# openjamoses/TOSEM-2021-Replication

Hardware: AMD Instinct MI355X
Metric: train_tokens_per_s (higher is better)
Workload: dtype bf16; 1 GPU; model=mltc-base, global_batch=128, seq_len=512, parallelism=dp1

## Files before the change

### csrc/flash_attn.hip

```cpp

#include "common.h"
#include "launchers.h"

typedef __attribute__((ext_vector_type(16))) float f32x16;
typedef __attribute__((ext_vector_type(2))) unsigned uint2_t;
typedef __attribute__((ext_vector_type(4))) unsigned uint4_t;

#define FA_DH 64
#define FA_KVB 32
#define FA_QB 32
#define FA_WAVES 4
#define FA_BLOCK (FA_WAVES * WAVE)
#define FA_QWG (FA_WAVES * FA_QB)
#define FA_Q2WG (2 * FA_QWG)

#define TILE_LDS_BYTES (FA_KVB * 128)
#define FWD_LDS_BYTES (2 * TILE_LDS_BYTES + FA_WAVES * 64 * sizeof(float))
#define BWD_LDS_BYTES (2 * TILE_LDS_BYTES + 64 * sizeof(float))
#define BWD_SEG_LDS_BYTES (BWD_LDS_BYTES + 32 * sizeof(int))
#define DQ_LDS_BYTES TILE_LDS_BYTES
#define DQR_LDS_BYTES (2 * TILE_LDS_BYTES + 16)

struct FaGeom {
  long qkv_bs, qkv_hs; int qkv_rs;
  long o_bs, o_hs; int o_rs;
  static FaGeom bhld(int H, int L) {
    return {(long)H * L * FA_DH, (long)L * FA_DH, FA_DH,
            (long)H * L * FA_DH, (long)L * FA_DH, FA_DH};
  }
  static FaGeom packed(int H, int L) {
    const int D = H * FA_DH;
    return {(long)L * 3 * D, 64L, 3 * D, (long)L * D, 64L, D};
  }
};


__device__ __forceinline__ int kswz(int row, int byte_off) {
  return byte_off ^ ((row & 7) << 4);
}

__device__ __forceinline__ int c_row(int r, int half) {
  return (r & 3) + 8 * (r >> 2) + 4 * half;
}

struct FaStager {
  int row, byte;
  __device__ __forceinline__ explicit FaStager(int tid)
      : row(tid >> 3), byte((tid & 7) * 16) {}
  __device__ __forceinline__ short8_t load(const short* base, int row0,
                                           int rs) const {
    return *(const short8_t*)(base + (long)(row0 + row) * rs + (byte >> 1));
  }
  __device__ __forceinline__ void store(short* lds, short8_t v) const {
    *(short8_t*)((char*)lds + row * 128 + kswz(row, byte)) = v;
  }
};

__device__ __forceinline__ short8_t tile_row_frag(const short* lds, int col,
                                                  int half, int c) {
  return *(const short8_t*)((const char*)lds + col * 128 +
                            kswz(col, (16 * c + 8 * half) * 2));
}

__device__ __forceinline__ void cvt_pk_swap(const float (&s)[16], int r0,
                                            int r1, uint4_t& u, int i) {
  unsigned lo, hi;
  asm("v_cvt_pk_bf16_f32 %0, %1, %2\n\ts_nop 1" : "=v"(lo)
      : "v"(s[r0]), "v"(s[r0 + 1]));
  asm("v_cvt_pk_bf16_f32 %0, %1, %2\n\ts_nop 1" : "=v"(hi)
      : "v"(s[r1]), "v"(s[r1 + 1]));
  auto sw = __builtin_amdgcn_permlane32_swap(lo, hi, false, false);
  u[i] = sw[0]; u[i + 2] = sw[1];
}

__device__ __forceinline__ void c_to_afrag2(const float (&sa)[16],
                                            short8_t (&fa)[2],
                                            const float (&sb)[16],
                                            short8_t (&fb)[2]) {
#pragma unroll
  for (int c = 0; c < 2; ++c) {
    uint4_t ua, ub;
#pragma unroll
    for (int i = 0; i < 2; ++i) {
      int r0 = c * 8 + 2 * i;
      int r1 = c * 8 + 4 + 2 * i;
      cvt_pk_swap(sa, r0, r1, ua, i);
      cvt_pk_swap(sb, r0, r1, ub, i);
    }
    fa[c] = __builtin_bit_cast(short8_t, ua);
    fb[c] = __builtin_bit_cast(short8_t, ub);
  }
}

struct FaTrFrags {
  uint2_t r[8];
  __device__ __forceinline__ short8_t frag(int c, int t) const {
    uint4_t w;
    w[0] = r[c * 4 + 0 * 2 + t][0];
    w[1] = r[c * 4 + 0 * 2 + t][1];
    w[2] = r[c * 4 + 1 * 2 + t][0];
    w[3] = r[c * 4 + 1 * 2 + t][1];
    return __builtin_bit_cast(short8_t, w);
  }
};

struct FaTrOffsets { unsigned a[8]; };

__device__ __forceinline__ FaTrOffsets tr_offsets(int lane, int half) {
  const int row_mate = (lane >> 2) & 3;
  const int d_lane = 16 * ((lane >> 4) & 1) + 4 * (lane & 3);
  FaTrOffsets o;
#pragma unroll
  for (int c = 0; c < 2; ++c)
#pragma unroll
    for (int rr = 0; rr < 2; ++rr)
#pragma unroll
      for (int t = 0; t < 2; ++t) {
        int row = 16 * c + 8 * half + 4 * rr + row_mate;
        int dcol = (32 * t + d_lane) * 2;
        o.a[c * 4 + rr * 2 + t] = row * 128 + kswz(row, dcol);
      }
  return o;
}

__device__ __forceinline__ void tr_issue(const short* lds,
                                         const FaTrOffsets& o, FaTrFrags& f) {
  const unsigned base = (unsigned)(unsigned long)(char*)lds;
  unsigned a[8];
#pragma unroll
  for (int i = 0; i < 8; ++i) a[i] = base + o.a[i];
  asm volatile(
      "ds_read_b64_tr_b16 %0, %8\n\t"
      "ds_read_b64_tr_b16 %1, %9\n\t"
      "ds_read_b64_tr_b16 %2, %10\n\t"
      "ds_read_b64_tr_b16 %3, %11\n\t"
      "ds_read_b64_tr_b16 %4, %12\n\t"
      "ds_read_b64_tr_b16 %5, %13\n\t"
      "ds_read_b64_tr_b16 %6, %14\n\t"
      "ds_read_b64_tr_b16 %7, %15\n\t"
      "s_waitcnt lgkmcnt(0)"
      : "=&v"(f.r[0]), "=&v"(f.r[1]), "=&v"(f.r[2]), "=&v"(f.r[3]),
        "=&v"(f.r[4]), "=&v"(f.r[5]), "=&v"(f.r[6]), "=&v"(f.r[7])
      : "v"(a[0]), "v"(a[1]), "v"(a[2]), "v"(a[3]), "v"(a[4]), "v"(a[5]),
        "v"(a[6]), "v"(a[7])
      : "memory");
}

__device__ __forceinline__ void tr_gather(const short* lds,
                                          const FaTrOffsets& o, FaTrFrags& f) {
  tr_issue(lds, o, f);
  __builtin_amdgcn_sched_barrier(0);
}

struct FaQBlocks { int bh, qA, qB; };

__device__ __forceinline__ FaQBlocks fa_qblocks(int L, int wid) {
  const int n_qblocks = (L + FA_Q2WG - 1) / FA_Q2WG;
  const int bid = xcd_group_remap(blockIdx.x, gridDim.x, n_qblocks);
  const int qA = (bid % n_qblocks) * FA_Q2WG + wid * FA_QB;
  return {bid / n_qblocks, qA, qA + FA_QWG};
}

__device__ __forceinline__ float fa_half_merge(float s) {
  return s + __shfl_xor(s, 32, WAVE);
}

__device__ __forceinline__ void fa_colsum_merge_store(const float* cs, int tid,
                                                      float* dst0,
                                                      float* dst1) {
  if (tid < 2 * FA_DH) {
    const int slot = tid / FA_DH, c = tid % FA_DH;
    const float* p = cs + slot * FA_WAVES * FA_DH + c;
    float s = p[0];
#pragma unroll
    for (int w = 1; w < FA_WAVES; ++w) s += p[w * FA_DH];
    float* dst = slot ? dst1 : dst0;
    if (dst) dst[c] = s;
  }
}

__device__ __forceinline__ int fa_last_active_kv(const float* mrow, int L,
                                                 int tid, int* scratch) {
  if (tid == 0) *scratch = -1;
  __syncthreads();
  int loc = -1;
  for (int kv = tid; kv < L; kv += FA_BLOCK)
    if (mrow[kv] > -1.0e8f) loc = kv;
  if (loc >= 0) atomicMax(scratch, loc);
  __syncthreads();
  return *scratch;
}

#define FA_SEG_BIAS -1.0e9f

struct FaRange { int lo, hi; };

__device__ __forceinline__ FaRange fa_seg_range(const int* srow, int L,
                                                int r_lo, int r_hi, int tid,
                                                int* scratch) {
  const int s_first = srow[r_lo], s_last = srow[r_hi];
  if (tid == 0) { scratch[0] = r_lo; scratch[1] = r_hi; }
  __syncthreads();
  int lo = r_lo, hi = r_hi;
  for (int j = tid; j < L; j += FA_BLOCK) {
    const int s = srow[j];
    if (s == s_first) lo = min(lo, j);
    if (s == s_last) hi = max(hi, j);
  }
  atomicMin(&scratch[0], lo);
  atomicMax(&scratch[1], hi);
  __syncthreads();
  return {scratch[0], scratch[1]};
}

__device__ __forceinline__ bool fa_seg_tile_live(const int (&r)[16], int a,
                                                 int b) {
  bool hit = false;
#pragma unroll
  for (int i = 0; i < 16; ++i) hit |= (r[i] == a) | (r[i] == b);
  return __builtin_amdgcn_ballot_w64(hit) != 0;
}

template <bool SEG>
__global__ void __launch_bounds__(FA_BLOCK, 2)
flash_fwd_kernel(const short* __restrict__ q, const short* __restrict__ k,
                 const short* __restrict__ v, const float* __restrict__ mask,
                 const int* __restrict__ seg,
                 short* __restrict__ o, float* __restrict__ lse,
                 int B, int H, int L, float scale, FaGeom g) {
  extern __shared__ __attribute__((aligned(16))) char smem[];
  short* k_lds = (short*)smem;
  short* v_lds = (short*)(smem + TILE_LDS_BYTES);
  float* alpha_lds = (float*)(smem + 2 * TILE_LDS_BYTES);

  const int tid = threadIdx.x;
  const int lane = tid & (WAVE - 1);
  const int wid = tid / WAVE;
  const int col = lane & 31;
  const int half = lane >> 5;
  const FaTrOffsets tro = tr_offsets(lane, half);

  const FaQBlocks qb = fa_qblocks(L, wid);
  const int b = qb.bh / H;
  const int h = qb.bh % H;
  const long qkv_off = (long)b * g.qkv_bs + (long)h * g.qkv_hs;
  const long o_off = (long)b * g.o_bs + (long)h * g.o_hs;
  const int my_qA = qb.qA + col;
  const int my_qB = qb.qB + col;
  const bool validA = my_qA < L;
  const bool validB = my_qB < L;
  const float* mrow = (!SEG && mask) ? mask + (long)b * L : nullptr;
  const int* srow = SEG ? seg + (long)b * L : nullptr;
  int sqA = 0, sqB = 0;
  if constexpr (SEG) {
    sqA = srow[validA ? my_qA : L - 1];
    sqB = srow[validB ? my_qB : L - 1];
  }

  short8_t qfA[4], qfB[4];
  {
    const short* qrA = q + qkv_off + (long)(validA ? my_qA : L - 1) * g.qkv_rs;
    const short* qrB = q + qkv_off + (long)(validB ? my_qB : L - 1) * g.qkv_rs;
#pragma unroll
    for (int c = 0; c < 4; ++c) {
      qfA[c] = *(const short8_t*)(qrA + c * 16 + half * 8);
      qfB[c] = *(const short8_t*)(qrB + c * 16 + half * 8);
    }
  }

  f32x16 oA[2], oB[2];
#pragma unroll
  for (int t = 0; t < 2; ++t) { oA[t] = (f32x16)(0.f); oB[t] = (f32x16)(0.f); }
  float mA = -3.0e38f, lA = 0.f, mB = -3.0e38f, lB = 0.f;

  const int n_kv = L / FA_KVB;
  int kt_begin = 0;
  int n_kv_eff = n_kv;
  if (mrow) {
    int last = fa_last_active_kv(mrow, L, tid, (int*)alpha_lds);
    if (last >= 0) n_kv_eff = min(n_kv, last / FA_KVB + 1);
  }
  if constexpr (SEG) {
    const int q_lo = qb.qA - wid * FA_QB;
    const FaRange kr = fa_seg_range(srow, L, q_lo, min(q_lo + FA_Q2WG, L) - 1,
                                    tid, (int*)alpha_lds);
    kt_begin = kr.lo / FA_KVB;
    n_kv_eff = kr.hi / FA_KVB + 1;
  }
  const FaStager st(tid);
  short8_t kv8 = st.load(k + qkv_off, kt_begin * FA_KVB, g.qkv_rs);
  short8_t vv8 = st.load(v + qkv_off, kt_begin * FA_KVB, g.qkv_rs);
  for (int kt = kt_begin; kt < n_kv_eff; ++kt) {
    const int kv0 = kt * FA_KVB;
    __syncthreads();
    st.store(k_lds, kv8);
    st.store(v_lds, vv8);
    __syncthreads();
    if (kt + 1 < n_kv_eff) {
      kv8 = st.load(k + qkv_off, kv0 + FA_KVB, g.qkv_rs);
      vv8 = st.load(v + qkv_off, kv0 + FA_KVB, g.qkv_rs);
    }

    float mb_r[16];
    int sk_r[16];
#pragma unroll
    for (int r = 0; r < 16; ++r) {
      if constexpr (SEG) sk_r[r] = srow[kv0 + c_row(r, half)];
      else mb_r[r] = mrow ? mrow[kv0 + c_row(r, half)] : 0.f;
    }
    if constexpr (SEG) {
      if (!fa_seg_tile_live(sk_r, sqA, sqB)) continue;
    }

    f32x16 sA = (f32x16)(0.f), sB = (f32x16)(0.f);
    __builtin_amdgcn_s_setprio(1);
#pragma unroll
    for (int c = 0; c < 4; ++c) {
      short8_t kf = tile_row_frag(k_lds, col, half, c);
      sA = __builtin_amdgcn_mfma_f32_32x32x16_bf16(kf, qfA[c], sA, 0, 0, 0);
      sB = __builtin_amdgcn_mfma_f32_32x32x16_bf16(kf, qfB[c], sB, 0, 0, 0);
    }
    __builtin_amdgcn_s_setprio(0);

    float svA[16], svB[16];
    float tmaxA = -3.0e38f, tmaxB = -3.0e38f;
#pragma unroll
    for (int r = 0; r < 16; ++r) {
      float mbA, mbB;
      if constexpr (SEG) {
        mbA = sk_r[r] == sqA ? 0.f : FA_SEG_BIAS;
        mbB = sk_r[r] == sqB ? 0.f : FA_SEG_BIAS;
      } else {
        mbA = mbB = mb_r[r];
      }
      float xA = sA[r] * scale + mbA;
      float xB = sB[r] * scale + mbB;
      svA[r] = xA; svB[r] = xB;
      tmaxA = fmaxf(tmaxA, xA);
      tmaxB = fmaxf(tmaxB, xB);
    }
    tmaxA = fmaxf(tmaxA, __shfl_xor(tmaxA, 32, WAVE));
    tmaxB = fmaxf(tmaxB, __shfl_xor(tmaxB, 32, WAVE));
    float mnA = fmaxf(mA, tmaxA), mnB = fmaxf(mB, tmaxB);
    float aA = __expf(mA - mnA), aB = __expf(mB - mnB);
    float rsA = 0.f, rsB = 0.f;
#pragma unroll
    for (int r = 0; r < 16; ++r) {
      svA[r] = __expf(svA[r] - mnA);
      svB[r] = __expf(svB[r] - mnB);
      rsA += svA[r];
      rsB += svB[r];
    }
    rsA += __shfl_xor(rsA, 32, WAVE);
    rsB += __shfl_xor(rsB, 32, WAVE);
    lA = lA * aA + rsA; mA = mnA;
    lB = lB * aB + rsB; mB = mnB;

    if (__builtin_amdgcn_ballot_w64(aA != 1.f || aB != 1.f)) {
      alpha_lds[wid * 64 + col] = aA;
      alpha_lds[wid * 64 + 32 + col] = aB;
#pragma unroll
      for (int t = 0; t < 2; ++t) {
#pragma unroll
        for (int r = 0; r < 16; ++r) {
          int qrow = c_row(r, half);
          oA[t][r] *= alpha_lds[wid * 64 + qrow];
          oB[t][r] *= alpha_lds[wid * 64 + 32 + qrow];
        }
      }
    }

    short8_t pfA[2], pfB[2];
    c_to_afrag2(svA, pfA, svB, pfB);

    FaTrFrags vT;
    tr_gather(v_lds, tro, vT);
    __builtin_amdgcn_s_setprio(1);
#pragma unroll
    for (int t = 0; t < 2; ++t) {
#pragma unroll
      for (int c = 0; c < 2; ++c) {
        short8_t vf = vT.frag(c, t);
        oA[t] = __builtin_amdgcn_mfma_f32_32x32x16_bf16(pfA[c], vf, oA[t],
                                                        0, 0, 0);
        oB[t] = __builtin_amdgcn_mfma_f32_32x32x16_bf16(pfB[c], vf, oB[t],
                                                        0, 0, 0);
      }
    }
    __builtin_amdgcn_s_setprio(0);
  }

  if (lse != nullptr && half == 0) {
    if (validA) lse[(long)qb.bh * L + my_qA] = mA + __logf(lA);
    if (validB) lse[(long)qb.bh * L + my_qB] = mB + __logf(lB);
  }
  const float invA = 1.0f / lA, invB = 1.0f / lB;
#pragma unroll
  for (int r = 0; r < 16; ++r) {
    int rloc = c_row(r, half);
    float iA = __shfl(invA, rloc, WAVE);
    float iB = __shfl(invB, rloc, WAVE);
    int qA = qb.qA + rloc, qB = qb.qB + rloc;
#pragma unroll
    for (int t = 0; t < 2; ++t) {
      if (qA < L)
        o[o_off + (long)qA * g.o_rs + 32 * t + col] =
            f32_to_bf16(oA[t][r] * iA);
      if (qB < L)
        o[o_off + (long)qB * g.o_rs + 32 * t + col] =
            f32_to_bf16(oB[t][r] * iB);
    }
  }
}

static int fa_row_blocks(int B, int L, int rows_per_wg) {
  return B * ((L + rows_per_wg - 1) / rows_per_wg);
}
static dim3 fa_grid(int B, int H, int L, int rows_per_wg) {
  return dim3(H * fa_row_blocks(B, L, rows_per_wg));
}

extern "C" int flash_bias_ws_rows(int B, int L) {
  return fa_row_blocks(B, L, FA_QWG);
}

static void fa_fwd_dispatch(const short* q, const short* k, const short* v,
                            const void* mask, const void* seg, void* o,
                            void* lse, int B, int H, int L, float scale,
                            FaGeom g, hipStream_t stream) {
  const dim3 grid = fa_grid(B, H, L, FA_Q2WG);
  if (seg)
    flash_fwd_kernel<true><<<grid, FA_BLOCK, FWD_LDS_BYTES, stream>>>(
        q, k, v, nullptr, (const int*)seg, (short*)o, (float*)lse, B, H, L,
        scale, g);
  else
    flash_fwd_kernel<false><<<grid, FA_BLOCK, FWD_LDS_BYTES, stream>>>(
        q, k, v, (const float*)mask, nullptr, (short*)o, (float*)lse, B, H, L,
        scale, g);
}

extern "C" hipError_t flash_fwd_launch(const void* q, const void* k,
                                       const void* v, const void* mask,
                                       const void* seg, void* o, void* lse,
                                       int B, int H, int L, float scale,
                                       hipStream_t stream) {
  fa_fwd_dispatch((const short*)q, (const short*)k, (const short*)v, mask,
                  seg, o, lse, B, H, L, scale, FaGeom::bhld(H, L), stream);
  return hipGetLastError();
}

extern "C" hipError_t flash_fwd_packed_launch(const void* qkv,
                                              const void* mask,
                                              const void* seg, void* o,
                                              void* lse, int B, int H, int L,
                                              float scale,
                                              hipStream_t stream) {
  const int D = H * FA_DH;
  fa_fwd_dispatch((const short*)qkv, (const short*)qkv + D,
                  (const short*)qkv + 2 * D, mask, seg, o, lse, B, H, L,
                  scale, FaGeom::packed(H, L), stream);
  return hipGetLastError();
}



template <bool SEG, bool BIAS>
__global__ void __launch_bounds__(FA_BLOCK, 2)
flash_bwd_fused_kernel(const short* __restrict__ q, const short* __restrict__ k,
                       const short* __restrict__ v,
                       const short* __restrict__ dout,
                       const float* __restrict__ mask,
                       const int* __restrict__ seg,
                       const float* __restrict__ lse,
                       const float* __restrict__ ddot,
                       short* __restrict__ ds, short* __restrict__ dk,
                       short* __restrict__ dv,
                       int B, int H, int L, float scale, FaGeom g,
                       float* __restrict__ bias_ws, int bias_ld) {
  extern __shared__ __attribute__((aligned(16))) char smem[];
  short* q_lds = (short*)smem;
  short* do_lds = (short*)(smem + TILE_LDS_BYTES);
  float* lse_lds = (float*)(smem + 2 * TILE_LDS_BYTES);
  float* dd_lds = lse_lds + 32;
  int* seg_lds = (int*)(dd_lds + 32);

  const int tid = threadIdx.x;
  const int lane = tid & (WAVE - 1);
  const int wid = tid / WAVE;
  const int col = lane & 31;
  const int half = lane >> 5;
  const FaTrOffsets tro = tr_offsets(lane, half);

  const int n_kvblocks = (L + FA_QWG - 1) / FA_QWG;
  int bid = xcd_group_remap(blockIdx.x, gridDim.x, n_kvblocks);
  int bh = bid / n_kvblocks;
  int kb = bid % n_kvblocks;
  const int b = bh / H;
  const int h = bh % H;
  const long qkv_off = (long)b * g.qkv_bs + (long)h * g.qkv_hs;
  const long o_off = (long)b * g.o_bs + (long)h * g.o_hs;
  const long bh_sq = (long)bh * L * L;
  const int kv_base = kb * FA_QWG + wid * FA_KVB;
  const int my_kv = kv_base + col;
  const bool kv_valid = my_kv < L;
  const float* mrow = (!SEG && mask) ? mask + (long)b * L : nullptr;
  const float mb = mrow ? mrow[min(my_kv, L - 1)] : 0.f;
  const int* srow = SEG ? seg + (long)b * L : nullptr;
  int sk = 0;
  if constexpr (SEG) sk = srow[min(my_kv, L - 1)];

  bool skip_tile = false;
  bool wave_skip = false;
  if (mrow && ds == nullptr) {
    int* any_lds = (int*)lse_lds;
    if (tid == 0) *any_lds = 0;
    __syncthreads();
    if (kv_valid && mb > -1.0e8f) *any_lds = 1;
    __syncthreads();
    skip_tile = (*any_lds == 0) && (mrow[0] > -1.0e8f);
    __syncthreads();
    wave_skip = !skip_tile && (mrow[0] > -1.0e8f) &&
        __builtin_amdgcn_ballot_w64(kv_valid && mb > -1.0e8f) == 0;
  }

  short8_t kf[4], vf[4];
  if (!skip_tile) {
    const short* kr = k + qkv_off + (long)(kv_valid ? my_kv : L - 1) * g.qkv_rs;
    const short* vr = v + qkv_off + (long)(kv_valid ? my_kv : L - 1) * g.qkv_rs;
#pragma unroll
    for (int c = 0; c < 4; ++c) {
      kf[c] = *(const short8_t*)(kr + c * 16 + half * 8);
      vf[c] = *(const short8_t*)(vr + c * 16 + half * 8);
    }
  }
  f32x16 dv_acc[2], dk_acc[2];
#pragma unroll
  for (int t = 0; t < 2; ++t) {
    dv_acc[t] = (f32x16)(0.f);
    dk_acc[t] = (f32x16)(0.f);
  }
  if (!skip_tile) {
  int qt_begin = 0;
  int n_q = L / 32;
  if constexpr (SEG) {
    const int kv_lo = kb * FA_QWG;
    const FaRange qr = fa_seg_range(srow, L, kv_lo, min(kv_lo + FA_QWG, L) - 1,
                                    tid, (int*)lse_lds);
    qt_begin = qr.lo / 32;
    n_q = qr.hi / 32 + 1;
  }
  const FaStager st(tid);
  short8_t qv8 = st.load(q + qkv_off, qt_begin * 32, g.qkv_rs);
  short8_t dv8 = st.load(dout + o_off, qt_begin * 32, g.o_rs);
  for (int qt = qt_begin; qt < n_q; ++qt) {
    const int q0 = qt * 32;
    __syncthreads();
    st.store(q_lds, qv8);
    st.store(do_lds, dv8);
    if (tid < 32) {
      lse_lds[tid] = lse[(long)bh * L + q0 + tid];
      dd_lds[tid] = ddot[(long)bh * L + q0 + tid];
      if constexpr (SEG) seg_lds[tid] = srow[q0 + tid];
    }
    __syncthreads();
    if (qt + 1 < n_q) {
      qv8 = st.load(q + qkv_off, q0 + 32, g.qkv_rs);
      dv8 = st.load(dout + o_off, q0 + 32, g.o_rs);
    }

    if (wave_skip) continue;
    int sq_r[16];
    if constexpr (SEG) {
#pragma unroll
      for (int r = 0; r < 16; ++r) sq_r[r] = seg_lds[c_row(r, half)];
      if (!fa_seg_tile_live(sq_r, sk, sk)) continue;
    }
    f32x16 s_acc = (f32x16)(0.f);
    f32x16 dp_acc = (f32x16)(0.f);
    __builtin_amdgcn_s_setprio(1);
#pragma unroll
    for (int c = 0; c < 4; ++c) {
      short8_t qfrag = tile_row_frag(q_lds, col, half, c);
      short8_t dofrag = tile_row_frag(do_lds, col, half, c);
      s_acc = __builtin_amdgcn_mfma_f32_32x32x16_bf16(qfrag, kf[c], s_acc,
                                                      0, 0, 0);
      dp_acc = __builtin_amdgcn_mfma_f32_32x32x16_bf16(dofrag, vf[c], dp_acc,
                                                       0, 0, 0);
    }
    __builtin_amdgcn_s_setprio(0);

    float pv[16], gv[16];
#pragma unroll
    for (int r = 0; r < 16; ++r) {
      int ql = c_row(r, half);
      float bias = mb;
      if constexpr (SEG) bias = sq_r[r] == sk ? 0.f : FA_SEG_BIAS;
      pv[r] = __expf(s_acc[r] * scale + bias - lse_lds[ql]);
      gv[r] = scale * pv[r] * (dp_acc[r] - dd_lds[ql]);
    }
    if (!SEG && ds != nullptr && kv_valid) {
#pragma unroll
      for (int r = 0; r < 16; ++r)
        ds[bh_sq + (long)(q0 + c_row(r, half)) * L + my_kv] =
            f32_to_bf16(gv[r]);
    }

    short8_t pf[2], gf[2];
    c_to_afrag2(pv, pf, gv, gf);

    FaTrFrags doT, qT;
    tr_issue(do_lds, tro, doT);
    tr_gather(q_lds, tro, qT);
    __builtin_amdgcn_s_setprio(1);
#pragma unroll
    for (int t = 0; t < 2; ++t) {
#pragma unroll
      for (int c = 0; c < 2; ++c) {
        dv_acc[t] = __builtin_amdgcn_mfma_f32_32x32x16_bf16(
            pf[c], doT.frag(c, t), dv_acc[t], 0, 0, 0);
        dk_acc[t] = __builtin_amdgcn_mfma_f32_32x32x16_bf16(
            gf[c], qT.frag(c, t), dk_acc[t], 0, 0, 0);
      }
    }
    __builtin_amdgcn_s_setprio(0);
  }
  }

  float csk[2] = {0.f, 0.f}, csv[2] = {0.f, 0.f};
#pragma unroll
  for (int t = 0; t < 2; ++t) {
#pragma unroll
    for (int r = 0; r < 16; ++r) {
      int kvl = c_row(r, half);
      if (kv_base + kvl >= L) continue;
      long off = qkv_off + (long)(kv_base + kvl) * g.qkv_rs + 32 * t + col;
      const short vb = f32_to_bf16(dv_acc[t][r]);
      const short kb16 = f32_to_bf16(dk_acc[t][r]);
      dv[off] = vb;
      dk[off] = kb16;
      if constexpr (BIAS) {
        csv[t] += bf16_to_f32(vb);
        csk[t] += bf16_to_f32(kb16);
      }
    }
  }
  if constexpr (BIAS) {
    float* cs = (float*)smem;
    __syncthreads();
#pragma unroll
    for (int t = 0; t < 2; ++t) {
      float sk_ = fa_half_merge(csk[t]);
      float sv_ = fa_half_merge(csv[t]);
      if (half == 0) {
        cs[(0 * FA_WAVES + wid) * FA_DH + 32 * t + col] = sk_;
        cs[(1 * FA_WAVES + wid) * FA_DH + 32 * t + col] = sv_;
      }
    }
    __syncthreads();
    const int third = bias_ld / 3;
    float* row = bias_ws + ((long)b * n_kvblocks + kb) * bias_ld + h * FA_DH;
    fa_colsum_merge_store(cs, tid, row + third, row + 2 * third);
  }
}

static void fa_bwd_fused_dispatch(const short* q, const short* k,
                                  const short* v, const void* dout,
                                  const void* mask, const void* seg,
                                  const void* lse, const void* ddot, void* ds,
                                  short* dk, short* dv, int B, int H, int L,
                                  float scale, FaGeom g, float* bias_ws,
                                  hipStream_t stream) {
  const dim3 grid = fa_grid(B, H, L, FA_QWG);
  const int bias_ld = 3 * H * FA_DH;
#define FA_BWD_SEG_ARGS                                                       \
  q, k, v, (const short*)dout, nullptr, (const int*)seg, (const float*)lse,   \
      (const float*)ddot, nullptr, dk, dv, B, H, L, scale, g, bias_ws, bias_ld
#define FA_BWD_ARGS                                                           \
  q, k, v, (const short*)dout, (const float*)mask, nullptr,                   \
      (const float*)lse, (const float*)ddot, (short*)ds, dk, dv, B, H, L,     \
      scale, g, bias_ws, bias_ld
  if (seg && bias_ws) {
    flash_bwd_fused_kernel<true, true><<<grid, FA_BLOCK, BWD_SEG_LDS_BYTES,
                                         stream>>>(FA_BWD_SEG_ARGS);
  } else if (seg) {
    flash_bwd_fused_kernel<true, false><<<grid, FA_BLOCK, BWD_SEG_LDS_BYTES,
                                          stream>>>(FA_BWD_SEG_ARGS);
  } else if (bias_ws) {
    flash_bwd_fused_kernel<false, true><<<grid, FA_BLOCK, BWD_LDS_BYTES,
                                          stream>>>(FA_BWD_ARGS);
  } else {
    flash_bwd_fused_kernel<false, false><<<grid, FA_BLOCK, BWD_LDS_BYTES,
                                           stream>>>(FA_BWD_ARGS);
  }
#undef FA_BWD_ARGS
#undef FA_BWD_SEG_ARGS
}

extern "C" hipError_t flash_bwd_fused_launch(
    const void* q, const void* k, const void* v, const void* dout,
    const void* mask, const void* seg, const void* lse, const void* ddot,
    void* ds, void* dk, void* dv, int B, int H, int L, float scale,
    hipStream_t stream) {
  if (seg && ds) return hipErrorInvalidValue;
  fa_bwd_fused_dispatch((const short*)q, (const short*)k, (const short*)v,
                        dout, mask, seg, lse, ddot, ds, (short*)dk,
                        (short*)dv, B, H, L, scale, FaGeom::bhld(H, L),
                        nullptr, stream);
  return hipGetLastError();
}

extern "C" hipError_t flash_bwd_fused_packed_launch(
    const void* qkv, const void* dout, const void* mask, const void* seg,
    const void* lse, const void* ddot, void* dqkv, void* bias_ws, int B,
    int H, int L, float scale, hipStream_t stream) {
  const int D = H * FA_DH;
  fa_bwd_fused_dispatch((const short*)qkv, (const short*)qkv + D,
                        (const short*)qkv + 2 * D, dout, mask, seg, lse, ddot,
                        nullptr, (short*)dqkv + D, (short*)dqkv + 2 * D, B, H,
                        L, scale, FaGeom::packed(H, L), (float*)bias_ws,
                        stream);
  return hipGetLastError();
}

extern "C" __global__ void __launch_bounds__(FA_BLOCK, 2)
flash_dq_kernel(const short* __restrict__ ds, const short* __restrict__ k,
                short* __restrict__ dq, int B, int H, int L) {
  extern __shared__ __attribute__((aligned(16))) char smem[];
  short* k_lds = (short*)smem;

  const int tid = threadIdx.x;
  const int lane = tid & (WAVE - 1);
  const int wid = tid / WAVE;
  const int col = lane & 31;
  const int half = lane >> 5;
  const FaTrOffsets tro = tr_offsets(lane, half);

  const FaQBlocks qb = fa_qblocks(L, wid);
  const long bh_off = (long)qb.bh * L * FA_DH;
  const long bh_sq = (long)qb.bh * L * L;
  const int my_qA = min(qb.qA + col, L - 1);
  const int my_qB = min(qb.qB + col, L - 1);
  const short* dsA_row = ds + bh_sq + (long)my_qA * L;
  const short* dsB_row = ds + bh_sq + (long)my_qB * L;

  f32x16 oA[2], oB[2];
#pragma unroll
  for (int t = 0; t < 2; ++t) { oA[t] = (f32x16)(0.f); oB[t] = (f32x16)(0.f); }

  const int n_kv = L / FA_KVB;
  const FaStager st(tid);
  short8_t kv8 = st.load(k + bh_off, 0, FA_DH);
  for (int kt = 0; kt < n_kv; ++kt) {
    const int kv0 = kt * FA_KVB;
    __syncthreads();
    st.store(k_lds, kv8);
    __syncthreads();
    if (kt + 1 < n_kv) kv8 = st.load(k + bh_off, kv0 + FA_KVB, FA_DH);
    short8_t aA[2], aB[2];
#pragma unroll
    for (int c = 0; c < 2; ++c) {
      aA[c] = *(const short8_t*)(dsA_row + kv0 + 16 * c + 8 * half);
      aB[c] = *(const short8_t*)(dsB_row + kv0 + 16 * c + 8 * half);
    }
    FaTrFrags kT;
    tr_gather(k_lds, tro, kT);
    __builtin_amdgcn_s_setprio(1);
#pragma unroll
    for (int t = 0; t < 2; ++t) {
#pragma unroll
      for (int c = 0; c < 2; ++c) {
        short8_t kf = kT.frag(c, t);
        oA[t] = __builtin_amdgcn_mfma_f32_32x32x16_bf16(aA[c], kf, oA[t],
                                                        0, 0, 0);
        oB[t] = __builtin_amdgcn_mfma_f32_32x32x16_bf16(aB[c], kf, oB[t],
                                                        0, 0, 0);
      }
    }
    __builtin_amdgcn_s_setprio(0);
  }

#pragma unroll
  for (int t = 0; t < 2; ++t) {
#pragma unroll
    for (int r = 0; r < 16; ++r) {
      int rloc = c_row(r, half);
      int qA = qb.qA + rloc, qB = qb.qB + rloc;
      if (qA < L)
        dq[bh_off + (long)qA * FA_DH + 32 * t + col] = f32_to_bf16(oA[t][r]);
      if (qB < L)
        dq[bh_off + (long)qB * FA_DH + 32 * t + col] = f32_to_bf16(oB[t][r]);
    }
  }
}

extern "C" hipError_t flash_dq_launch(const void* ds, const void* k, void* dq,
                                      int B, int H, int L,
                                      hipStream_t stream) {
  flash_dq_kernel<<<fa_grid(B, H, L, FA_Q2WG), FA_BLOCK, DQ_LDS_BYTES,
                    stream>>>(
      (const short*)ds, (const short*)k, (short*)dq, B, H, L);
  return hipGetLastError();
}

template <bool SEG, bool BIAS>
__global__ void __launch_bounds__(FA_BLOCK, 2)
flash_dq_recompute_kernel(const short* __restrict__ q,
                          const short* __restrict__ k,
                          const short* __restrict__ v,
                          const short* __restrict__ dout,
                          const float* __restrict__ mask,
                          const int* __restrict__ seg,
                          const float* __restrict__ lse,
                          const float* __restrict__ ddot,
                          short* __restrict__ dq,
                          int B, int H, int L, float scale, FaGeom g,
                          float* __restrict__ bias_ws, int bias_ld) {
  extern __shared__ __attribute__((aligned(16))) char smem[];
  short* k_lds = (short*)smem;
  short* v_lds = (short*)(smem + TILE_LDS_BYTES);
  int* skip_scratch = (int*)(smem + 2 * TILE_LDS_BYTES);

  const int tid = threadIdx.x;
  const int lane = tid & (WAVE - 1);
  const int wid = tid / WAVE;
  const int col = lane & 31;
  const int half = lane >> 5;
  const FaTrOffsets tro = tr_offsets(lane, half);

  const FaQBlocks qb = fa_qblocks(L, wid);
  const int b = qb.bh / H;
  const int h = qb.bh % H;
  const long qkv_off = (long)b * g.qkv_bs + (long)h * g.qkv_hs;
  const long o_off = (long)b * g.o_bs + (long)h * g.o_hs;
  const int my_qA = qb.qA + col;
  const int my_qB = qb.qB + col;
  const bool validA = my_qA < L;
  const bool validB = my_qB < L;
  const float* mrow = (!SEG && mask) ? mask + (long)b * L : nullptr;
  const int* srow = SEG ? seg + (long)b * L : nullptr;
  int sqA = 0, sqB = 0;
  if constexpr (SEG) {
    sqA = srow[validA ? my_qA : L - 1];
    sqB = srow[validB ? my_qB : L - 1];
  }

  short8_t qfA[4], qfB[4], dofA[4], dofB[4];
  {
    const short* qrA = q + qkv_off + (long)(validA ? my_qA : L - 1) * g.qkv_rs;
    const short* qrB = q + qkv_off + (long)(validB ? my_qB : L - 1) * g.qkv_rs;
    const short* drA = dout + o_off + (long)(validA ? my_qA : L - 1) * g.o_rs;
    const short* drB = dout + o_off + (long)(validB ? my_qB : L - 1) * g.o_rs;
#pragma unroll
    for (int c = 0; c < 4; ++c) {
      qfA[c] = *(const short8_t*)(qrA + c * 16 + half * 8);
      qfB[c] = *(const short8_t*)(qrB + c * 16 + half * 8);
      dofA[c] = *(const short8_t*)(drA + c * 16 + half * 8);
      dofB[c] = *(const short8_t*)(drB + c * 16 + half * 8);
    }
  }
  const float lseA = lse[(long)qb.bh * L + (validA ? my_qA : L - 1)];
  const float lseB = lse[(long)qb.bh * L + (validB ? my_qB : L - 1)];
  const float ddA = ddot[(long)qb.bh * L + (validA ? my_qA : L - 1)];
  const float ddB = ddot[(long)qb.bh * L + (validB ? my_qB : L - 1)];

  f32x16 dqA[2], dqB[2];
#pragma unroll
  for (int t = 0; t < 2; ++t) { dqA[t] = (f32x16)(0.f); dqB[t] = (f32x16)(0.f); }

  const int n_kv = L / FA_KVB;
  int kt_begin = 0;
  int n_kv_eff = n_kv;
  if (mrow) {
    int last = fa_last_active_kv(mrow, L, tid, skip_scratch);
    if (last >= 0) n_kv_eff = min(n_kv, last / FA_KVB + 1);
  }
  if constexpr (SEG) {
    const int q_lo = qb.qA - wid * FA_QB;
    const FaRange kr = fa_seg_range(srow, L, q_lo, min(q_lo + FA_Q2WG, L) - 1,
                                    tid, skip_scratch);
    kt_begin = kr.lo / FA_KVB;
    n_kv_eff = kr.hi / FA_KVB + 1;
  }
  const FaStager st(tid);
  short8_t kv8 = st.load(k + qkv_off, kt_begin * FA_KVB, g.qkv_rs);
  short8_t vv8 = st.load(v + qkv_off, kt_begin * FA_KVB, g.qkv_rs);
  for (int kt = kt_begin; kt < n_kv_eff; ++kt) {
    const int kv0 = kt * FA_KVB;
    __syncthreads();
    st.store(k_lds, kv8);
    st.store(v_lds, vv8);
    __syncthreads();
    if (kt + 1 < n_kv_eff) {
      kv8 = st.load(k + qkv_off, kv0 + FA_KVB, g.qkv_rs);
      vv8 = st.load(v + qkv_off, kv0 + FA_KVB, g.qkv_rs);
    }

    float mb_r[16];
    int sk_r[16];
#pragma unroll
    for (int r = 0; r < 16; ++r) {
      if constexpr (SEG) sk_r[r] = srow[kv0 + c_row(r, half)];
      else mb_r[r] = mrow ? mrow[kv0 + c_row(r, half)] : 0.f;
    }
    if constexpr (SEG) {
      if (!fa_seg_tile_live(sk_r, sqA, sqB)) continue;
    }

    f32x16 sA = (f32x16)(0.f), sB = (f32x16)(0.f);
    f32x16 pA = (f32x16)(0.f), pB = (f32x16)(0.f);
    __builtin_amdgcn_s_setprio(1);
#pragma unroll
    for (int c = 0; c < 4; ++c) {
      short8_t kf = tile_row_frag(k_lds, col, half, c);
      short8_t vf = tile_row_frag(v_lds, col, half, c);
      sA = __builtin_amdgcn_mfma_f32_32x32x16_bf16(kf, qfA[c], sA, 0, 0, 0);
      sB = __builtin_amdgcn_mfma_f32_32x32x16_bf16(kf, qfB[c], sB, 0, 0, 0);
      pA = __builtin_amdgcn_mfma_f32_32x32x16_bf16(vf, dofA[c], pA, 0, 0, 0);
      pB = __builtin_amdgcn_mfma_f32_32x32x16_bf16(vf, dofB[c], pB, 0, 0, 0);
    }
    __builtin_amdgcn_s_setprio(0);

    float gA[16], gB[16];
#pragma unroll
    for (int r = 0; r < 16; ++r) {
      float mbA, mbB;
      if constexpr (SEG) {
        mbA = sk_r[r] == sqA ? 0.f : FA_SEG_BIAS;
        mbB = sk_r[r] == sqB ? 0.f : FA_SEG_BIAS;
      } else {
        mbA = mbB = mb_r[r];
      }
      float expA = __expf(sA[r] * scale + mbA - lseA);
      float expB = __expf(sB[r] * scale + mbB - lseB);
      gA[r] = scale * expA * (pA[r] - ddA);
      gB[r] = scale * expB * (pB[r] - ddB);
    }

    short8_t gfA[2], gfB[2];
    c_to_afrag2(gA, gfA, gB, gfB);

    FaTrFrags kT;
    tr_gather(k_lds, tro, kT);
    __builtin_amdgcn_s_setprio(1);
#pragma unroll
    for (int t = 0; t < 2; ++t) {
#pragma unroll
      for (int c = 0; c < 2; ++c) {
        short8_t kf = kT.frag(c, t);
        dqA[t] = __builtin_amdgcn_mfma_f32_32x32x16_bf16(gfA[c], kf, dqA[t],
                                                         0, 0, 0);
        dqB[t] = __builtin_amdgcn_mfma_f32_32x32x16_bf16(gfB[c], kf, dqB[t],
                                                         0, 0, 0);
      }
    }
    __builtin_amdgcn_s_setprio(0);
  }

  float csA[2] = {0.f, 0.f}, csB[2] = {0.f, 0.f};
#pragma unroll
  for (int t = 0; t < 2; ++t) {
#pragma unroll
    for (int r = 0; r < 16; ++r) {
      int rloc = c_row(r, half);
      int qA = qb.qA + rloc, qB = qb.qB + rloc;
      if (qA < L) {
        const short a16 = f32_to_bf16(dqA[t][r]);
        dq[qkv_off + (long)qA * g.qkv_rs + 32 * t + col] = a16;
        if constexpr (BIAS) csA[t] += bf16_to_f32(a16);
      }
      if (qB < L) {
        const short b16 = f32_to_bf16(dqB[t][r]);
        dq[qkv_off + (long)qB * g.qkv_rs + 32 * t + col] = b16;
        if constexpr (BIAS) csB[t] += bf16_to_f32(b16);
      }
    }
  }
  if constexpr (BIAS) {
    float* cs = (float*)smem;
    __syncthreads();
#pragma unroll
    for (int t = 0; t < 2; ++t) {
      float sA_ = fa_half_merge(csA[t]);
      float sB_ = fa_half_merge(csB[t]);
      if (half == 0) {
        cs[(0 * FA_WAVES + wid) * FA_DH + 32 * t + col] = sA_;
        cs[(1 * FA_WAVES + wid) * FA_DH + 32 * t + col] = sB_;
      }
    }
    __syncthreads();
    const int n128 = (L + FA_QWG - 1) / FA_QWG;
    const int blkA = (qb.qA - wid * FA_QB) / FA_QWG;
    float* row = bias_ws + ((long)b * n128 + blkA) * bias_ld + h * FA_DH;
    fa_colsum_merge_store(cs, tid, row,
                          blkA + 1 < n128 ? row + bias_ld : nullptr);
  }
}

static void fa_dq_recompute_dispatch(const short* q, const short* k,
                                     const short* v, const void* dout,
                                     const void* mask, const void* seg,
                                     const void* lse, const void* ddot,
                                     void* dq, int B, int H, int L,
                                     float scale, FaGeom g, float* bias_ws,
                                     hipStream_t stream) {
  const dim3 grid = fa_grid(B, H, L, FA_Q2WG);
  const int bias_ld = 3 * H * FA_DH;
#define FA_DQR_SEG_ARGS                                                       \
  q, k, v, (const short*)dout, nullptr, (const int*)seg, (const float*)lse,   \
      (const float*)ddot, (short*)dq, B, H, L, scale, g, bias_ws, bias_ld
#define FA_DQR_ARGS                                                           \
  q, k, v, (const short*)dout, (const float*)mask, nullptr,                   \
      (const float*)lse, (const float*)ddot, (short*)dq, B, H, L, scale, g,   \
      bias_ws, bias_ld
  if (seg && bias_ws) {
    flash_dq_recompute_kernel<true, true><<<grid, FA_BLOCK, DQR_LDS_BYTES,
                                            stream>>>(FA_DQR_SEG_ARGS);
  } else if (seg) {
    flash_dq_recompute_kernel<true, false><<<grid, FA_BLOCK, DQR_LDS_BYTES,
                                             stream>>>(FA_DQR_SEG_ARGS);
  } else if (bias_ws) {
    flash_dq_recompute_kernel<false, true><<<grid, FA_BLOCK, DQR_LDS_BYTES,
                                             stream>>>(FA_DQR_ARGS);
  } else {
    flash_dq_recompute_kernel<false, false><<<grid, FA_BLOCK, DQR_LDS_BYTES,
                                              stream>>>(FA_DQR_ARGS);
  }
#undef FA_DQR_ARGS
#undef FA_DQR_SEG_ARGS
}

extern "C" hipError_t flash_dq_recompute_launch(
    const void* q, const void* k, const void* v, const void* dout,
    const void* mask, const void* seg, const void* lse, const void* ddot,
    void* dq, int B, int H, int L, float scale, hipStream_t stream) {
  fa_dq_recompute_dispatch((const short*)q, (const short*)k, (const short*)v,
                           dout, mask, seg, lse, ddot, dq, B, H, L, scale,
                           FaGeom::bhld(H, L), nullptr, stream);
  return hipGetLastError();
}

extern "C" hipError_t flash_dq_recompute_packed_launch(
    const void* qkv, const void* dout, const void* mask, const void* seg,
    const void* lse, const void* ddot, void* dqkv, void* bias_ws, int B,
    int H, int L, float scale, hipStream_t stream) {
  const int D = H * FA_DH;
  fa_dq_recompute_dispatch((const short*)qkv, (const short*)qkv + D,
                           (const short*)qkv + 2 * D, dout, mask, seg, lse,
                           ddot, dqkv, B, H, L, scale, FaGeom::packed(H, L),
                           (float*)bias_ws, stream);
  return hipGetLastError();
}

__device__ __forceinline__ float fa_row_dot(const short* dr, const short* orow,
                                            int sub) {
  short4_t a = *(const short4_t*)(dr + sub * 4);
  short4_t c = *(const short4_t*)(orow + sub * 4);
  float s = 0.f;
#pragma unroll
  for (int j = 0; j < 4; ++j) s += bf16_to_f32(a[j]) * bf16_to_f32(c[j]);
#pragma unroll
  for (int off = 8; off > 0; off >>= 1) s += __shfl_xor(s, off, 16);
  return s;
}

extern "C" __global__ void __launch_bounds__(256)
fa_dot_kernel(const short* __restrict__ dout, const short* __restrict__ o,
              float* __restrict__ ddot, long n_rows) {
  long row = ((long)blockIdx.x * 256 + threadIdx.x) >> 4;
  if (row >= n_rows) return;
  int sub = threadIdx.x & 15;
  float s = fa_row_dot(dout + row * FA_DH, o + row * FA_DH, sub);
  if (sub == 0) ddot[row] = s;
}

extern "C" __global__ void __launch_bounds__(256)
fa_dot_packed_kernel(const short* __restrict__ dout,
                     const short* __restrict__ o, float* __restrict__ ddot,
                     int B, int H, int L) {
  const int D = H * FA_DH;
  long n_rows = (long)B * L * H;
  long chunk = ((long)blockIdx.x * 256 + threadIdx.x) >> 4;
  if (chunk >= n_rows) return;
  int sub = threadIdx.x & 15;
  int h = (int)(chunk % H);
  long bl = chunk / H;
  int l = (int)(bl % L);
  int b = (int)(bl / L);
  float s = fa_row_dot(dout + bl * D + h * FA_DH, o + bl * D + h * FA_DH, sub);
  if (sub == 0) ddot[((long)b * H + h) * L + l] = s;
}

extern "C" hipError_t fa_dot_packed_launch(const void* dout, const void* o,
                                           void* ddot, int B, int H, int L,
                                           hipStream_t stream) {
  long total_threads = (long)B * H * L * 16;
  int grid = (int)((total_threads + 255) / 256);
  fa_dot_packed_kernel<<<grid, 256, 0, stream>>>(
      (const short*)dout, (const short*)o, (float*)ddot, B, H, L);
  return hipGetLastError();
}

extern "C" hipError_t fa_dot_launch(const void* dout, const void* o,
                                    void* ddot, long n_rows,
                                    hipStream_t stream) {
  long total_threads = n_rows * 16;
  int grid = (int)((total_threads + 255) / 256);
  fa_dot_kernel<<<grid, 256, 0, stream>>>((const short*)dout, (const short*)o,
                                          (float*)ddot, n_rows);
  return hipGetLastError();
}

extern "C" __global__ void __launch_bounds__(64)
tr_probe_kernel(const short* __restrict__ src, short* __restrict__ out,
                int scheme) {
  __shared__ __attribute__((aligned(16))) short lds[256];
  int lane = threadIdx.x;
  for (int i = lane; i < 256; i += 64) lds[i] = src[i];
  __syncthreads();
  int addr;
  switch (scheme) {
    case 0: addr = 0; break;
    case 1: addr = (lane & 15) * 2; break;
    case 2: addr = ((lane & 15) + (lane >> 4) * 64) * 2; break;
    case 3: addr = (lane >> 4) * 128; break;
    case 4: addr = (lane & 3) * 16; break;
    case 5: addr = ((lane & 3) * 32 + 4 * ((lane >> 2) & 7)) * 2; break;
    case 6: addr = ((lane & 3) * 8 + 4) * 2; break;
    case 7: addr = ((lane & 3) == 0) ? 16 : 0; break;
    case 8: addr = ((lane & 3) == 1) ? 16 : 0; break;
    case 9: addr = ((lane & 3) == 2) ? 16 : 0; break;
    case 10: addr = ((lane & 3) == 3) ? 16 : 0; break;
    case 11: addr = ((lane & 3) * 64 + 4 * ((lane >> 2) & 7)) * 2; break;
    default: addr = ((lane & 3) * 8 + ((lane >> 2) & 7) * 32) * 2; break;
  }
  typedef __attribute__((ext_vector_type(2))) unsigned uint2_t;
  uint2_t r;
  unsigned base = (unsigned)(unsigned long)((char*)lds + addr);
  asm volatile("ds_read_b64_tr_b16 %0, %1\n\ts_waitcnt lgkmcnt(0)"
               : "=v"(r) : "v"(base) : "memory");
  __builtin_amdgcn_sched_barrier(0);
  out[lane * 4 + 0] = (short)(r[0] & 0xffff);
  out[lane * 4 + 1] = (short)(r[0] >> 16);
  out[lane * 4 + 2] = (short)(r[1] & 0xffff);
  out[lane * 4 + 3] = (short)(r[1] >> 16);
}

extern "C" hipError_t tr_probe_launch(const void* src, void* out, int scheme,
                                      hipStream_t stream) {
  tr_probe_kernel<<<1, 64, 0, stream>>>((const short*)src, (short*)out,
                                        scheme);
  return hipGetLastError();
}
```

### csrc/launchers.h

```cpp
#pragma once

#include <hip/hip_runtime.h>

extern "C" {

hipError_t ln_fwd_launch(const void* x, const void* res, const void* gamma,
                         const void* beta, void* y, void* s_out, void* mean,
                         void* rstd, int N, int D, float eps,
                         hipStream_t stream);
hipError_t ln_bwd_launch(const void* dy, const void* x, const void* gamma,
                         const void* mean, const void* rstd,
                         const void* ds_extra, void* dx, void* ws, int n_out,
                         int N, int D, hipStream_t stream);
int ln_bwd_ws_rows(int N, int D);
hipError_t ln_drop_fwd_launch(const void* x, const void* res,
                              const void* gamma, const void* beta, void* y,
                              void* s_out, void* mean, void* rstd, int N,
                              int D, float eps, unsigned long long seed,
                              unsigned call, unsigned site, unsigned thr,
                              hipStream_t stream);
hipError_t ln_drop_bwd_launch(const void* dy, const void* x,
                              const void* gamma, const void* mean,
                              const void* rstd, const void* ds_extra, void* dx,
                              void* dres, void* ws, int N, int D,
                              unsigned long long seed, unsigned call,
                              unsigned site, unsigned thr,
                              hipStream_t stream);
int ln_drop_bwd_max_d(void);

hipError_t colsum_launch(const void* ws, void* scratch, void* out, int R,
                         int D, int split_w, int out_bf16,
                         hipStream_t stream);
int colsum_scratch_rows(void);
hipError_t colsum_bf16_launch(const void* x, void* scratch, void* out, long N,
                              int D, hipStream_t stream);
int colsum_bf16_scratch_rows(void);

hipError_t bias_gelu_fwd_launch(const void* x, const void* b, void* y,
                                long n_elem, int D, hipStream_t stream);
hipError_t bias_gelu_bwd_launch(const void* dy, const void* x, const void* b,
                                void* dx, void* ws_dbias, long n_elem, int D,
                                hipStream_t stream);
int bias_gelu_bwd_ws_rows(long n_elem, int D);

hipError_t softmax_fwd_launch(const void* s, const void* mask, void* p,
                              long n_rows, int Lk, int H_Lq, float scale,
                              hipStream_t stream);
hipError_t softmax_bwd_launch(const void* dp, const void* p, void* ds,
                              long n_rows, int Lk, float scale,
                              hipStream_t stream);
hipError_t p_from_lse_launch(const void* s, const void* mask, const void* lse,
                             void* p, long n_rows, int Lk, int H_Lq,
                             float scale, hipStream_t stream);

hipError_t adamw_launch(void* p_bf16, const void* grad, int grad_is_f32,
                        void* m, void* v, void* master, long n, float lr,
                        float beta1, float beta2, float eps, float wd,
                        int step, float grad_scale, hipStream_t stream);
hipError_t adamw_clipped_launch(void* p_bf16, const void* grad,
                                int grad_is_f32, void* m, void* v,
                                void* master, long n, float lr, float beta1,
                                float beta2, float eps, float wd, int step,
                                const void* clip_state, hipStream_t stream);
hipError_t grad_clip_state_launch(const void* grad, int grad_is_f32, long n,
                                  float grad_scale, float max_norm,
                                  void* partials, void* clip_state,
                                  hipStream_t stream);
int grad_norm_grid(long n);

hipError_t qkv_repack_launch(const void* src, void* dst, int B, int L, int H,
                             int dh, int backward, hipStream_t stream);
hipError_t qkv_repack_bwd3_launch(const void* dq, const void* dk,
                                  const void* dv, void* dsrc, int B, int L,
                                  int H, int dh, hipStream_t stream);
hipError_t out_repack_launch(const void* src, void* dst, int B, int L, int H,
                             int dh, int backward, hipStream_t stream);

hipError_t flash_fwd_launch(const void* q, const void* k, const void* v,
                            const void* mask, const void* seg, void* o,
                            void* lse, int B, int H, int L, float scale,
                            hipStream_t stream);
hipError_t flash_fwd_packed_launch(const void* qkv, const void* mask,
                                   const void* seg, void* o, void* lse, int B,
                                   int H, int L, float scale,
                                   hipStream_t stream);
hipError_t flash_bwd_fused_launch(const void* q, const void* k, const void* v,
                                  const void* dout, const void* mask,
                                  const void* seg, const void* lse,
                                  const void* ddot, void* ds, void* dk,
                                  void* dv, int B, int H, int L, float scale,
                                  hipStream_t stream);
hipError_t flash_bwd_fused_packed_launch(const void* qkv, const void* dout,
                                         const void* mask, const void* seg,
                                         const void* lse, const void* ddot,
                                         void* dqkv, void* bias_ws, int B,
                                         int H, int L, float scale,
                                         hipStream_t stream);
hipError_t flash_dq_recompute_packed_launch(const void* qkv, const void* dout,
                                            const void* mask, const void* seg,
                                            const void* lse, const void* ddot,
                                            void* dqkv, void* bias_ws, int B,
                                            int H, int L, float scale,
                                            hipStream_t stream);
int flash_bias_ws_rows(int B, int L);
hipError_t flash_dq_recompute_launch(const void* q, const void* k,
                                     const void* v, const void* dout,
                                     const void* mask, const void* seg,
                                     const void* lse, const void* ddot,
                                     void* dq, int B, int H, int L,
                                     float scale, hipStream_t stream);
hipError_t flash_dq_launch(const void* ds, const void* k, void* dq, int B,
                           int H, int L, hipStream_t stream);
hipError_t fa_dot_launch(const void* dout, const void* o, void* ddot,
                         long n_rows, hipStream_t stream);
hipError_t fa_dot_packed_launch(const void* dout, const void* o, void* ddot,
                                int B, int H, int L, hipStream_t stream);
hipError_t tr_probe_launch(const void* src, void* out, int scheme,
                           hipStream_t stream);

hipError_t masked_pool_fwd_launch(const void* x, const void* mask,
                                  void* pooled, void* counts, void* ws, int B,
                                  int L, int D, hipStream_t stream);
int masked_pool_ws_splits(void);
hipError_t masked_pool_bwd_launch(const void* dpooled, const void* mask,
                                  const void* counts, void* dx, int B, int L,
                                  int D, hipStream_t stream);
hipError_t segment_pool_fwd_launch(const void* x, const void* seg_start,
                                   const void* seg_len, void* pooled, int N,
                                   long T, int D, hipStream_t stream);
hipError_t segment_pool_bwd_launch(const void* dpooled, const void* pos2seg,
                                   const void* seg_len, void* dx, int N,
                                   long T, int D, hipStream_t stream);

hipError_t wgrad_gemm_launch(const void* a, const void* b, void* ws, void* out,
                             int M, int N, long K, int S, hipStream_t stream);

}
```

### csrc/ops.cpp

```cpp

#include <torch/extension.h>
#include <c10/hip/HIPStream.h>
#include <hip/hip_runtime.h>

#include "launchers.h"
#include "lt_gemm.h"

namespace {

#define CHECK_HIP(call)                                                   \
  do {                                                                    \
    hipError_t e_ = (call);                                               \
    TORCH_CHECK(e_ == hipSuccess, "HIP error: ", hipGetErrorString(e_));  \
  } while (0)

hipStream_t cur_stream() {
  return c10::hip::getCurrentHIPStream().stream();
}

void check_bf16(const torch::Tensor& t, const char* name) {
  TORCH_CHECK(t.is_contiguous(), name, " must be contiguous");
  TORCH_CHECK(t.scalar_type() == torch::kBFloat16, name, " must be bf16");
  TORCH_CHECK(t.device().is_cuda(), name, " must be on GPU");
}

void check_f32(const torch::Tensor& t, const char* name) {
  TORCH_CHECK(t.is_contiguous(), name, " must be contiguous");
  TORCH_CHECK(t.scalar_type() == torch::kFloat32, name, " must be f32");
  TORCH_CHECK(t.device().is_cuda(), name, " must be on GPU");
}

void check_shape(const torch::Tensor& t, const char* name,
                 at::IntArrayRef want, const char* shape) {
  TORCH_CHECK(t.sizes() == want, name, " must be ", shape);
}

void check_numel(const torch::Tensor& t, const char* name, long n,
                 const char* shape) {
  TORCH_CHECK(t.numel() == n, name, " must be ", shape);
}

void check_mult8(long v, const char* name) {
  TORCH_CHECK(v % 8 == 0, name, " must be a multiple of 8, got ", v);
}

const void* softmax_mask_ptr(const c10::optional<torch::Tensor>& mask,
                             const torch::Tensor& scores, int* H_Lq) {
  *H_Lq = 1;
  if (!mask.has_value()) return nullptr;
  check_f32(*mask, "mask");
  TORCH_CHECK(scores.dim() == 4, "masked scores must be [B, H, Lq, Lk]");
  check_shape(*mask, "mask", {scores.size(0), scores.size(3)}, "[B, Lk]");
  *H_Lq = (int)(scores.size(1) * scores.size(2));
  return mask->data_ptr();
}

const void* pool_mask_ptr(const c10::optional<torch::Tensor>& mask,
                          const torch::Tensor& x, long B, long L) {
  if (!mask.has_value()) return nullptr;
  TORCH_CHECK(mask->scalar_type() == torch::kBool && mask->is_contiguous(),
              "mask must be contiguous bool");
  TORCH_CHECK(mask->device() == x.device(), "mask must be on the same device "
              "as the data");
  check_shape(*mask, "mask", {B, L}, "[B, L]");
  return mask->data_ptr();
}

torch::Tensor colsum(const torch::Tensor& ws, long split_w, bool out_bf16) {
  const long R = ws.size(0), W = ws.size(1);
  auto out = torch::empty(
      {W}, out_bf16 ? ws.options().dtype(torch::kBFloat16) : ws.options());
  auto scratch = torch::empty({colsum_scratch_rows(), W}, ws.options());
  CHECK_HIP(colsum_launch(ws.data_ptr(), scratch.data_ptr(), out.data_ptr(),
                          (int)R, (int)W, (int)split_w, out_bf16 ? 1 : 0,
                          cur_stream()));
  return out;
}


struct FlashDims { long B, H, L; };
using NamedTensor = std::pair<const char*, torch::Tensor>;

const void* flash_mask_ptr(const c10::optional<torch::Tensor>& mask,
                           const FlashDims& d) {
  if (!mask.has_value()) return nullptr;
  check_f32(*mask, "mask");
  TORCH_CHECK(mask->dim() == 2 && mask->size(0) == d.B &&
              mask->size(1) == d.L, "mask must be [B, L]");
  return mask->data_ptr();
}

const void* flash_seg_ptr(const c10::optional<torch::Tensor>& seg,
                          const c10::optional<torch::Tensor>& mask,
                          const torch::Tensor& x, const FlashDims& d) {
  if (!seg.has_value()) return nullptr;
  TORCH_CHECK(!mask.has_value(), "mask and seg are mutually exclusive");
  TORCH_CHECK(seg->scalar_type() == torch::kInt32, "seg must be int32");
  TORCH_CHECK(seg->device() == x.device(), "seg must be on the same device "
              "as the attention inputs");
  TORCH_CHECK(seg->is_contiguous(), "seg must be contiguous");
  TORCH_CHECK(seg->dim() == 2 && seg->size(0) == d.B && seg->size(1) == d.L,
              "seg must be [B, L]");
  return seg->data_ptr();
}

void check_i32(const torch::Tensor& t, const torch::Tensor& like,
               const char* name) {
  TORCH_CHECK(t.is_contiguous(), name, " must be contiguous");
  TORCH_CHECK(t.scalar_type() == torch::kInt32, name, " must be int32");
  TORCH_CHECK(t.device() == like.device(), name, " must be on the same "
              "device as the data");
}

void check_flash_rows(std::initializer_list<NamedTensor> rows,
                      const FlashDims& d) {
  for (const auto& [name, t] : rows) {
    check_f32(t, name);
    TORCH_CHECK(t.dim() == 3 && t.size(0) == d.B && t.size(1) == d.H &&
                t.size(2) == d.L, name, " must be [B, H, L]");
  }
}

FlashDims check_flash_bhld(const char* xname, const torch::Tensor& x,
                           std::initializer_list<NamedTensor> same,
                           std::initializer_list<NamedTensor> rows) {
  check_bf16(x, xname);
  TORCH_CHECK(x.dim() == 4, xname, " must be [B, H, L, 64]");
  const FlashDims d{x.size(0), x.size(1), x.size(2)};
  TORCH_CHECK(x.size(3) == 64, "flash kernels are specialized for head_dim 64");
  TORCH_CHECK(d.L % 32 == 0, "flash kernels need L % 32 == 0");
  for (const auto& [name, t] : same) {
    check_bf16(t, name);
    TORCH_CHECK(t.sizes() == x.sizes(), name, " must match ", xname,
                "'s shape");
  }
  check_flash_rows(rows, d);
  return d;
}

FlashDims check_flash_packed(const torch::Tensor& qkv, long H,
                             std::initializer_list<NamedTensor> outs,
                             std::initializer_list<NamedTensor> rows) {
  check_bf16(qkv, "qkv");
  TORCH_CHECK(qkv.dim() == 3, "qkv must be [B, L, 3D]");
  const FlashDims d{qkv.size(0), H, qkv.size(1)};
  TORCH_CHECK(qkv.size(2) == 3 * H * 64, "qkv last dim must be 3*H*64");
  TORCH_CHECK(d.L % 32 == 0, "flash kernels need L % 32 == 0");
  for (const auto& [name, t] : outs) {
    check_bf16(t, name);
    TORCH_CHECK(t.dim() == 3 && t.size(0) == d.B && t.size(1) == d.L &&
                t.size(2) == H * 64, name, " must be [B, L, H*64]");
  }
  check_flash_rows(rows, d);
  return d;
}

}

std::vector<torch::Tensor> layernorm_fwd(torch::Tensor x,
                                         c10::optional<torch::Tensor> residual,
                                         torch::Tensor gamma,
                                         torch::Tensor beta, double eps) {
  check_bf16(x, "x"); check_bf16(gamma, "gamma"); check_bf16(beta, "beta");
  const int D = (int)x.size(-1);
  const long N = x.numel() / D;
  TORCH_CHECK(D % 8 == 0, "D must be a multiple of 8, got ", D);
  check_numel(gamma, "gamma", D, "[D]");
  check_numel(beta, "beta", D, "[D]");
  if (residual.has_value()) {
    check_bf16(*residual, "residual");
    TORCH_CHECK(residual->sizes() == x.sizes(), "residual shape mismatch");
  }
  auto y = torch::empty_like(x);
  auto opts = x.options().dtype(torch::kFloat32);
  auto mean = torch::empty({N}, opts);
  auto rstd = torch::empty({N}, opts);
  const void* res_ptr = nullptr;
  torch::Tensor s_out;
  void* s_ptr = nullptr;
  if (residual.has_value()) {
    res_ptr = residual->data_ptr();
    s_out = torch::empty_like(x);
    s_ptr = s_out.data_ptr();
  } else {
    s_out = x;
  }
  CHECK_HIP(ln_fwd_launch(x.data_ptr(), res_ptr, gamma.data_ptr(),
                          beta.data_ptr(), y.data_ptr(), s_ptr,
                          mean.data_ptr(), rstd.data_ptr(), (int)N, D,
                          (float)eps, cur_stream()));
  return {y, s_out, mean, rstd};
}

std::vector<torch::Tensor> layernorm_bwd(torch::Tensor dy, torch::Tensor x,
                                         torch::Tensor gamma, torch::Tensor mean,
                                         torch::Tensor rstd,
                                         c10::optional<torch::Tensor> ds_extra,
                                         bool want_dres, bool out_bf16) {
  check_bf16(dy, "dy"); check_bf16(x, "x"); check_bf16(gamma, "gamma");
  const int D = (int)x.size(-1);
  const long N = x.numel() / D;
  TORCH_CHECK(D % 8 == 0, "D must be a multiple of 8, got ", D);
  TORCH_CHECK(dy.numel() == x.numel(), "dy shape mismatch");
  check_numel(gamma, "gamma", D, "[D]");
  check_f32(mean, "mean"); check_f32(rstd, "rstd");
  TORCH_CHECK(mean.numel() == N && rstd.numel() == N,
              "mean and rstd must be [N]");
  const void* de = nullptr;
  if (ds_extra.has_value()) {
    check_bf16(*ds_extra, "ds_extra");
    TORCH_CHECK(ds_extra->numel() == x.numel(), "ds_extra shape mismatch");
    de = ds_extra->data_ptr();
  }
  auto dx = torch::empty_like(x);
  const int n_out = want_dres ? 3 : 2;
  auto ws = torch::empty({ln_bwd_ws_rows((int)N, D), n_out * D},
                         x.options().dtype(torch::kFloat32));
  CHECK_HIP(ln_bwd_launch(dy.data_ptr(), x.data_ptr(), gamma.data_ptr(),
                          mean.data_ptr(), rstd.data_ptr(), de, dx.data_ptr(),
                          ws.data_ptr(), n_out, (int)N, D, cur_stream()));
  auto cols = colsum(ws, 2 * D, out_bf16);
  std::vector<torch::Tensor> out = {dx, cols.narrow(0, 0, D),
                                    cols.narrow(0, D, D)};
  if (want_dres) out.push_back(cols.narrow(0, 2 * D, D));
  return out;
}

void check_drop_args(int64_t call, int64_t site, int64_t thr) {
  TORCH_CHECK(call >= 0 && call <= 0xffffffffLL, "call must fit 32 bits");
  TORCH_CHECK(site >= 0 && site <= 0xffffffffLL, "site must fit 32 bits");
  TORCH_CHECK(thr >= 1 && thr <= 65535,
              "dropout threshold must be in [1, 65535], got ", thr);
}

std::vector<torch::Tensor> layernorm_drop_fwd(torch::Tensor x,
                                              torch::Tensor residual,
                                              torch::Tensor gamma,
                                              torch::Tensor beta, double eps,
                                              uint64_t seed, int64_t call,
                                              int64_t site, int64_t thr) {
  check_bf16(x, "x"); check_bf16(gamma, "gamma"); check_bf16(beta, "beta");
  check_bf16(residual, "residual");
  const int D = (int)x.size(-1);
  const long N = x.numel() / D;
  TORCH_CHECK(D % 8 == 0, "D must be a multiple of 8, got ", D);
  check_numel(gamma, "gamma", D, "[D]");
  check_numel(beta, "beta", D, "[D]");
  TORCH_CHECK(residual.sizes() == x.sizes(), "residual shape mismatch");
  TORCH_CHECK(D <= ln_drop_bwd_max_d(), "fused dropout LayerNorm supports "
              "D <= ", ln_drop_bwd_max_d(), ", got ", D);
  check_drop_args(call, site, thr);
  auto y = torch::empty_like(x);
  auto s_out = torch::empty_like(x);
  auto opts = x.options().dtype(torch::kFloat32);
  auto mean = torch::empty({N}, opts);
  auto rstd = torch::empty({N}, opts);
  CHECK_HIP(ln_drop_fwd_launch(x.data_ptr(), residual.data_ptr(),
                               gamma.data_ptr(), beta.data_ptr(), y.data_ptr(),
                               s_out.data_ptr(), mean.data_ptr(),
                               rstd.data_ptr(), (int)N, D, (float)eps, seed,
                               (unsigned)call, (unsigned)site, (unsigned)thr,
                               cur_stream()));
  return {y, s_out, mean, rstd};
}

std::vector<torch::Tensor> layernorm_drop_bwd(
    torch::Tensor dy, torch::Tensor x, torch::Tensor gamma, torch::Tensor mean,
    torch::Tensor rstd, c10::optional<torch::Tensor> ds_extra, bool out_bf16,
    uint64_t seed, int64_t call, int64_t site, int64_t thr) {
  check_bf16(dy, "dy"); check_bf16(x, "x"); check_bf16(gamma, "gamma");
  const int D = (int)x.size(-1);
  const long N = x.numel() / D;
  TORCH_CHECK(D % 8 == 0, "D must be a multiple of 8, got ", D);
  TORCH_CHECK(D <= ln_drop_bwd_max_d(), "fused dropout LayerNorm backward "
              "supports D <= ", ln_drop_bwd_max_d(), ", got ", D);
  TORCH_CHECK(dy.numel() == x.numel(), "dy shape mismatch");
  check_numel(gamma, "gamma", D, "[D]");
  check_f32(mean, "mean"); check_f32(rstd, "rstd");
  TORCH_CHECK(mean.numel() == N && rstd.numel() == N,
              "mean and rstd must be [N]");
  check_drop_args(call, site, thr);
  const void* de = nullptr;
  if (ds_extra.has_value()) {
    check_bf16(*ds_extra, "ds_extra");
    TORCH_CHECK(ds_extra->numel() == x.numel(), "ds_extra shape mismatch");
    de = ds_extra->data_ptr();
  }
  auto dx = torch::empty_like(x);
  auto dres = torch::empty_like(x);
  auto ws = torch::empty({ln_bwd_ws_rows((int)N, D), 2 * D},
                         x.options().dtype(torch::kFloat32));
  CHECK_HIP(ln_drop_bwd_launch(dy.data_ptr(), x.data_ptr(), gamma.data_ptr(),
                               mean.data_ptr(), rstd.data_ptr(), de,
                               dx.data_ptr(), dres.data_ptr(), ws.data_ptr(),
                               (int)N, D, seed, (unsigned)call, (unsigned)site,
                               (unsigned)thr, cur_stream()));
  auto cols = colsum(ws, 2 * D, out_bf16);
  return {dx, dres, cols.narrow(0, 0, D), cols.narrow(0, D, D)};
}

torch::Tensor bias_gelu_fwd(torch::Tensor x, torch::Tensor b) {
  check_bf16(x, "x"); check_bf16(b, "b");
  const int D = (int)x.size(-1);
  const long n = x.numel();
  TORCH_CHECK(D % 8 == 0, "D must be a multiple of 8");
  check_numel(b, "b", D, "[D]");
  auto y = torch::empty_like(x);
  CHECK_HIP(bias_gelu_fwd_launch(x.data_ptr(), b.data_ptr(), y.data_ptr(), n,
                                 D, cur_stream()));
  return y;
}

std::vector<torch::Tensor> bias_gelu_bwd(torch::Tensor dy, torch::Tensor x,
                                         torch::Tensor b, bool out_bf16) {
  check_bf16(dy, "dy"); check_bf16(x, "x"); check_bf16(b, "b");
  const int D = (int)x.size(-1);
  const long n = x.numel();
  TORCH_CHECK(D % 8 == 0, "D must be a multiple of 8");
  check_numel(b, "b", D, "[D]");
  TORCH_CHECK(dy.numel() == x.numel(), "dy shape mismatch");
  auto dx = torch::empty_like(x);
  auto ws = torch::empty({bias_gelu_bwd_ws_rows(n, D), D},
                         x.options().dtype(torch::kFloat32));
  CHECK_HIP(bias_gelu_bwd_launch(dy.data_ptr(), x.data_ptr(), b.data_ptr(),
                                 dx.data_ptr(), ws.data_ptr(), n, D,
                                 cur_stream()));
  return {dx, colsum(ws, D, out_bf16)};
}

torch::Tensor softmax_fwd(torch::Tensor scores, c10::optional<torch::Tensor> mask,
                          double scale) {
  check_bf16(scores, "scores");
  const int Lk = (int)scores.size(-1);
  const long n_rows = scores.numel() / Lk;
  check_mult8(Lk, "Lk");
  int H_Lq;
  const void* mptr = softmax_mask_ptr(mask, scores, &H_Lq);
  auto p = torch::empty_like(scores);
  CHECK_HIP(softmax_fwd_launch(scores.data_ptr(), mptr, p.data_ptr(), n_rows,
                               Lk, H_Lq, (float)scale, cur_stream()));
  return p;
}

torch::Tensor softmax_bwd(torch::Tensor dp, torch::Tensor p, double scale) {
  check_bf16(dp, "dp"); check_bf16(p, "p");
  const int Lk = (int)p.size(-1);
  const long n_rows = p.numel() / Lk;
  check_mult8(Lk, "Lk");
  TORCH_CHECK(dp.sizes() == p.sizes(), "dp must match p's shape");
  auto ds = torch::empty_like(p);
  CHECK_HIP(softmax_bwd_launch(dp.data_ptr(), p.data_ptr(), ds.data_ptr(),
                               n_rows, Lk, (float)scale, cur_stream()));
  return ds;
}

void adamw_step(torch::Tensor p, torch::Tensor grad, torch::Tensor m,
                torch::Tensor v, torch::Tensor master, double lr, double beta1,
                double beta2, double eps, double wd, long step,
                double grad_scale) {
  check_bf16(p, "p"); check_f32(m, "m"); check_f32(v, "v");
  check_f32(master, "master");
  TORCH_CHECK(grad.is_contiguous() && grad.device().is_cuda(), "bad grad");
  int gf32 = grad.scalar_type() == torch::kFloat32;
  TORCH_CHECK(gf32 || grad.scalar_type() == torch::kBFloat16,
              "grad must be f32 or bf16");
  const long n = p.numel();
  TORCH_CHECK(n % 4 == 0, "flat parameter buffer must be padded to 4 elems");
  TORCH_CHECK(grad.numel() == n && m.numel() == n && v.numel() == n &&
              master.numel() == n, "size mismatch");
  CHECK_HIP(adamw_launch(p.data_ptr(), grad.data_ptr(), gf32, m.data_ptr(),
                         v.data_ptr(), master.data_ptr(), n, (float)lr,
                         (float)beta1, (float)beta2, (float)eps, (float)wd,
                         (int)step, (float)grad_scale, cur_stream()));
}

int check_flat_grad(const torch::Tensor& grad) {
  TORCH_CHECK(grad.is_contiguous() && grad.device().is_cuda(), "bad grad");
  int gf32 = grad.scalar_type() == torch::kFloat32;
  TORCH_CHECK(gf32 || grad.scalar_type() == torch::kBFloat16,
              "grad must be f32 or bf16");
  TORCH_CHECK(grad.numel() > 0 && grad.numel() % 8 == 0,
              "flat gradient buffer must be padded to 8 elems");
  TORCH_CHECK(reinterpret_cast<uintptr_t>(grad.data_ptr()) % 16 == 0,
              "flat gradient buffer must be 16-byte aligned");
  return gf32;
}

torch::Tensor grad_clip_state(torch::Tensor grad, double grad_scale,
                              double max_norm) {
  int gf32 = check_flat_grad(grad);
  TORCH_CHECK(max_norm > 0, "max_norm must be greater than 0");
  const long n = grad.numel();
  auto opts = torch::TensorOptions().dtype(torch::kFloat32)
                  .device(grad.device());
  auto partials = torch::empty({grad_norm_grid(n)}, opts);
  auto state = torch::empty({4}, opts);
  CHECK_HIP(grad_clip_state_launch(grad.data_ptr(), gf32, n,
                                   (float)grad_scale, (float)max_norm,
                                   partials.data_ptr(), state.data_ptr(),
                                   cur_stream()));
  return state;
}

void adamw_step_clipped(torch::Tensor p, torch::Tensor grad, torch::Tensor m,
                        torch::Tensor v, torch::Tensor master, double lr,
                        double beta1, double beta2, double eps, double wd,
                        long step, torch::Tensor clip_state) {
  check_bf16(p, "p"); check_f32(m, "m"); check_f32(v, "v");
  check_f32(master, "master"); check_f32(clip_state, "clip_state");
  int gf32 = check_flat_grad(grad);
  TORCH_CHECK(clip_state.numel() == 4, "clip_state must hold 4 floats");
  const long n = p.numel();
  TORCH_CHECK(grad.numel() == n && m.numel() == n && v.numel() == n &&
              master.numel() == n, "size mismatch");
  CHECK_HIP(adamw_clipped_launch(p.data_ptr(), grad.data_ptr(), gf32,
                                 m.data_ptr(), v.data_ptr(),
                                 master.data_ptr(), n, (float)lr,
                                 (float)beta1, (float)beta2, (float)eps,
                                 (float)wd, (int)step, clip_state.data_ptr(),
                                 cur_stream()));
}

torch::Tensor qkv_repack(torch::Tensor qkv, long H, bool backward) {
  check_bf16(qkv, "qkv");
  TORCH_CHECK(H > 0, "H must be positive");
  long B, L, dh;
  if (!backward) {
    TORCH_CHECK(qkv.dim() == 3 || qkv.dim() == 5,
                "qkv must be [B, L, 3*H*dh] or [B, L, 3, H, dh]");
    B = qkv.size(0); L = qkv.size(1);
    if (qkv.dim() == 3) {
      TORCH_CHECK(qkv.size(2) % (3 * H) == 0,
                  "qkv last dim must divide evenly by 3*H");
      dh = qkv.size(2) / (3 * H);
    } else {
      check_shape(qkv, "qkv", {B, L, 3, H, qkv.size(4)}, "[B, L, 3, H, dh]");
      dh = qkv.size(4);
    }
  } else {
    TORCH_CHECK(qkv.dim() == 5, "qkv grad must be [3, B, H, L, dh]");
    B = qkv.size(1); L = qkv.size(3);
    dh = qkv.size(4);
    check_shape(qkv, "qkv grad", {3, B, H, L, dh}, "[3, B, H, L, dh]");
  }
  check_mult8(dh, "head_dim");
  auto out = backward ? torch::empty({B, L, 3 * H * dh}, qkv.options())
                      : torch::empty({3, B, H, L, dh}, qkv.options());
  CHECK_HIP(qkv_repack_launch(qkv.data_ptr(), out.data_ptr(), (int)B, (int)L,
                              (int)H, (int)dh, backward ? 1 : 0,
                              cur_stream()));
  return out;
}

torch::Tensor qkv_repack_bwd3(torch::Tensor dq, torch::Tensor dk,
                              torch::Tensor dv) {
  check_bf16(dq, "dq"); check_bf16(dk, "dk"); check_bf16(dv, "dv");
  TORCH_CHECK(dq.dim() == 4, "dq must be [B, H, L, dh]");
  TORCH_CHECK(dk.sizes() == dq.sizes(), "dk must match dq's shape");
  TORCH_CHECK(dv.sizes() == dq.sizes(), "dv must match dq's shape");
  long B = dq.size(0), H = dq.size(1), L = dq.size(2), dh = dq.size(3);
  check_mult8(dh, "head_dim");
  auto out = torch::empty({B, L, 3 * H * dh}, dq.options());
  CHECK_HIP(qkv_repack_bwd3_launch(dq.data_ptr(), dk.data_ptr(), dv.data_ptr(),
                                   out.data_ptr(), (int)B, (int)L, (int)H,
                                   (int)dh, cur_stream()));
  return out;
}

torch::Tensor out_repack(torch::Tensor x, bool backward) {
  check_bf16(x, "x");
  TORCH_CHECK(!backward,
              "pass the 4-D grad with explicit dims via out_repack_bwd");
  TORCH_CHECK(x.dim() == 4, "x must be [B, H, L, dh]");
  long B = x.size(0), H = x.size(1), L = x.size(2), dh = x.size(3);
  check_mult8(dh, "head_dim");
  auto out = torch::empty({B, L, H * dh}, x.options());
  CHECK_HIP(out_repack_launch(x.data_ptr(), out.data_ptr(), (int)B, (int)L,
                              (int)H, (int)dh, 0, cur_stream()));
  return out;
}

torch::Tensor out_repack_bwd(torch::Tensor dgrad, long H) {
  check_bf16(dgrad, "dgrad");
  TORCH_CHECK(dgrad.dim() == 3, "dgrad must be [B, L, H*dh]");
  TORCH_CHECK(H > 0 && dgrad.size(2) % H == 0,
              "dgrad last dim must divide evenly by H");
  long B = dgrad.size(0), L = dgrad.size(1), dh = dgrad.size(2) / H;
  check_mult8(dh, "head_dim");
  auto out = torch::empty({B, H, L, dh}, dgrad.options());
  CHECK_HIP(out_repack_launch(dgrad.data_ptr(), out.data_ptr(), (int)B,
                              (int)L, (int)H, (int)dh, 1, cur_stream()));
  return out;
}

std::vector<torch::Tensor> flash_fwd(torch::Tensor q, torch::Tensor k,
                                     torch::Tensor v,
                                     c10::optional<torch::Tensor> mask,
                                     double scale,
                                     c10::optional<torch::Tensor> seg) {
  const auto [B, H, L] = check_flash_bhld("q", q, {{"k", k}, {"v", v}}, {});
  const void* mptr = flash_mask_ptr(mask, {B, H, L});
  const void* sptr = flash_seg_ptr(seg, mask, q, {B, H, L});
  auto o = torch::empty_like(q);
  auto lse = torch::empty({B, H, L}, q.options().dtype(torch::kFloat32));
  CHECK_HIP(flash_fwd_launch(q.data_ptr(), k.data_ptr(), v.data_ptr(), mptr,
                             sptr, o.data_ptr(), lse.data_ptr(), (int)B,
                             (int)H, (int)L, (float)scale, cur_stream()));
  return {o, lse};
}

torch::Tensor p_from_lse(torch::Tensor scores, c10::optional<torch::Tensor> mask,
                         torch::Tensor lse, double scale) {
  check_bf16(scores, "scores"); check_f32(lse, "lse");
  const int Lk = (int)scores.size(-1);
  const long n_rows = scores.numel() / Lk;
  TORCH_CHECK(lse.numel() == n_rows, "lse size mismatch");
  check_mult8(Lk, "Lk");
  int H_Lq;
  const void* mptr = softmax_mask_ptr(mask, scores, &H_Lq);
  auto p = torch::empty_like(scores);
  CHECK_HIP(p_from_lse_launch(scores.data_ptr(), mptr, lse.data_ptr(),
                              p.data_ptr(), n_rows, Lk, H_Lq, (float)scale,
                              cur_stream()));
  return p;
}

torch::Tensor fa_dot(torch::Tensor dout, torch::Tensor o) {
  check_bf16(dout, "dout"); check_bf16(o, "o");
  TORCH_CHECK(dout.dim() == 4 && o.sizes() == dout.sizes(),
              "dout and o must both be [B, H, L, 64]");
  const long n_rows = dout.numel() / dout.size(-1);
  TORCH_CHECK(dout.size(-1) == 64, "fa_dot expects head_dim 64");
  auto d = torch::empty({n_rows}, dout.options().dtype(torch::kFloat32));
  CHECK_HIP(fa_dot_launch(dout.data_ptr(), o.data_ptr(), d.data_ptr(), n_rows,
                          cur_stream()));
  return d.view({dout.size(0), dout.size(1), dout.size(2)});
}

std::vector<torch::Tensor> flash_bwd_fused(torch::Tensor q, torch::Tensor k,
                                           torch::Tensor v, torch::Tensor dout,
                                           c10::optional<torch::Tensor> mask,
                                           torch::Tensor lse,
                                           torch::Tensor ddot, double scale,
                                           bool emit_ds,
                                           c10::optional<torch::Tensor> seg) {
  const auto [B, H, L] = check_flash_bhld(
      "q", q, {{"k", k}, {"v", v}, {"dout", dout}},
      {{"lse", lse}, {"ddot", ddot}});
  const void* mptr = flash_mask_ptr(mask, {B, H, L});
  const void* sptr = flash_seg_ptr(seg, mask, q, {B, H, L});
  TORCH_CHECK(!(sptr && emit_ds), "seg with emit_ds=True is not supported: "
              "the flash_dq A/B path is unsegmented");
  auto dk = torch::empty_like(k);
  auto dv = torch::empty_like(v);
  torch::Tensor ds;
  void* ds_ptr = nullptr;
  if (emit_ds) {
    ds = torch::empty({B, H, L, L}, q.options());
    ds_ptr = ds.data_ptr();
  }
  CHECK_HIP(flash_bwd_fused_launch(q.data_ptr(), k.data_ptr(), v.data_ptr(),
                                   dout.data_ptr(), mptr, sptr,
                                   lse.data_ptr(), ddot.data_ptr(), ds_ptr,
                                   dk.data_ptr(), dv.data_ptr(), (int)B,
                                   (int)H, (int)L, (float)scale,
                                   cur_stream()));
  if (emit_ds) return {ds, dk, dv};
  return {dk, dv};
}

torch::Tensor wgrad_gemm(torch::Tensor dy, torch::Tensor x,
                         long splits) {
  check_bf16(dy, "dy"); check_bf16(x, "x");
  TORCH_CHECK(dy.dim() == 2 && x.dim() == 2, "2-D operands required");
  const long K = dy.size(0), M = dy.size(1), N = x.size(1);
  TORCH_CHECK(x.size(0) == K, "K mismatch");
  TORCH_CHECK(M % 256 == 0 && N % 256 == 0, "M, N must be 256-multiples");
  TORCH_CHECK(K % 32 == 0, "K must be a 32-multiple");
  int S = (int)splits;
  if (S <= 0) {
    long tiles = (M / 256) * (N / 256);
    S = 1;
    while (S < 32 && tiles * S < 512 && (K / (2L * S)) % 32 == 0) S *= 2;
  }
  TORCH_CHECK((K / S) % 32 == 0, "K/S must be a 32-multiple");
  auto ws = torch::empty({S, M, N}, dy.options().dtype(torch::kFloat32));
  auto out = torch::empty({M, N}, dy.options());
  CHECK_HIP(wgrad_gemm_launch(dy.data_ptr(), x.data_ptr(), ws.data_ptr(),
                              out.data_ptr(), (int)M, (int)N, K, S,
                              cur_stream()));
  return out;
}

torch::Tensor bias_grad(torch::Tensor dy) {
  check_bf16(dy, "dy");
  const int D = (int)dy.size(-1);
  const long N = dy.numel() / D;
  TORCH_CHECK(dy.dim() == 2, "dy must be [N, D]");
  TORCH_CHECK(D % 8 == 0, "D % 8 == 0 required");
  auto scratch = torch::empty({colsum_bf16_scratch_rows(), D},
                              dy.options().dtype(torch::kFloat32));
  auto out = torch::empty({D}, dy.options());
  CHECK_HIP(colsum_bf16_launch(dy.data_ptr(), scratch.data_ptr(),
                               out.data_ptr(), N, D, cur_stream()));
  return out;
}

std::vector<torch::Tensor> flash_fwd_packed(torch::Tensor qkv, long H,
                                            c10::optional<torch::Tensor> mask,
                                            double scale,
                                            c10::optional<torch::Tensor> seg) {
  const auto dims = check_flash_packed(qkv, H, {}, {});
  const long B = dims.B, L = dims.L;
  const void* mptr = flash_mask_ptr(mask, dims);
  const void* sptr = flash_seg_ptr(seg, mask, qkv, dims);
  auto o = torch::empty({B, L, H * 64}, qkv.options());
  auto lse = torch::empty({B, H, L}, qkv.options().dtype(torch::kFloat32));
  CHECK_HIP(flash_fwd_packed_launch(qkv.data_ptr(), mptr, sptr, o.data_ptr(),
                                    lse.data_ptr(), (int)B, (int)H, (int)L,
                                    (float)scale, cur_stream()));
  return {o, lse};
}

namespace {

std::vector<torch::Tensor> flash_bwd_packed_impl(
    torch::Tensor qkv, torch::Tensor o, torch::Tensor dout,
    c10::optional<torch::Tensor> mask, torch::Tensor lse, long H,
    double scale, c10::optional<torch::Tensor> seg, bool want_bias) {
  const auto dims = check_flash_packed(qkv, H, {{"o", o}, {"dout", dout}},
                                       {{"lse", lse}});
  const long B = dims.B, L = dims.L;
  const void* mptr = flash_mask_ptr(mask, dims);
  const void* sptr = flash_seg_ptr(seg, mask, qkv, dims);
  auto ddot = torch::empty({B, H, L}, qkv.options().dtype(torch::kFloat32));
  CHECK_HIP(fa_dot_packed_launch(dout.data_ptr(), o.data_ptr(),
                                 ddot.data_ptr(), (int)B, (int)H, (int)L,
                                 cur_stream()));
  auto dqkv = torch::empty_like(qkv);
  torch::Tensor ws;
  void* ws_ptr = nullptr;
  if (want_bias) {
    ws = torch::empty({flash_bias_ws_rows((int)B, (int)L), 3 * H * 64},
                      qkv.options().dtype(torch::kFloat32));
    ws_ptr = ws.data_ptr();
  }
  CHECK_HIP(flash_bwd_fused_packed_launch(
      qkv.data_ptr(), dout.data_ptr(), mptr, sptr, lse.data_ptr(),
      ddot.data_ptr(), dqkv.data_ptr(), ws_ptr, (int)B, (int)H, (int)L,
      (float)scale, cur_stream()));
  CHECK_HIP(flash_dq_recompute_packed_launch(
      qkv.data_ptr(), dout.data_ptr(), mptr, sptr, lse.data_ptr(),
      ddot.data_ptr(), dqkv.data_ptr(), ws_ptr, (int)B, (int)H, (int)L,
      (float)scale, cur_stream()));
  if (!want_bias) return {dqkv};
  return {dqkv, colsum(ws, ws.size(1), true)};
}

}

torch::Tensor flash_bwd_packed(torch::Tensor qkv, torch::Tensor o,
                               torch::Tensor dout,
                               c10::optional<torch::Tensor> mask,
                               torch::Tensor lse, long H, double scale,
                               c10::optional<torch::Tensor> seg) {
  return flash_bwd_packed_impl(qkv, o, dout, mask, lse, H, scale, seg,
                               false)[0];
}

std::vector<torch::Tensor> flash_bwd_packed_bias(
    torch::Tensor qkv, torch::Tensor o, torch::Tensor dout,
    c10::optional<torch::Tensor> mask, torch::Tensor lse, long H,
    double scale, c10::optional<torch::Tensor> seg) {
  return flash_bwd_packed_impl(qkv, o, dout, mask, lse, H, scale, seg, true);
}

torch::Tensor flash_dq_recompute(torch::Tensor q, torch::Tensor k,
                                 torch::Tensor v, torch::Tensor dout,
                                 c10::optional<torch::Tensor> mask,
                                 torch::Tensor lse, torch::Tensor ddot,
                                 double scale,
                                 c10::optional<torch::Tensor> seg) {
  const auto [B, H, L] = check_flash_bhld(
      "q", q, {{"k", k}, {"v", v}, {"dout", dout}},
      {{"lse", lse}, {"ddot", ddot}});
  const void* mptr = flash_mask_ptr(mask, {B, H, L});
  const void* sptr = flash_seg_ptr(seg, mask, q, {B, H, L});
  auto dq = torch::empty_like(q);
  CHECK_HIP(flash_dq_recompute_launch(q.data_ptr(), k.data_ptr(),
                                      v.data_ptr(), dout.data_ptr(), mptr,
                                      sptr, lse.data_ptr(), ddot.data_ptr(),
                                      dq.data_ptr(), (int)B, (int)H, (int)L,
                                      (float)scale, cur_stream()));
  return dq;
}

torch::Tensor flash_dq(torch::Tensor ds, torch::Tensor k) {
  const auto [B, H, L] = check_flash_bhld("k", k, {}, {});
  check_bf16(ds, "ds");
  TORCH_CHECK(ds.dim() == 4 && ds.size(0) == B && ds.size(1) == H &&
              ds.size(2) == L && ds.size(3) == L, "ds must be [B, H, L, L]");
  auto dq = torch::empty_like(k);
  CHECK_HIP(flash_dq_launch(ds.data_ptr(), k.data_ptr(), dq.data_ptr(),
                            (int)B, (int)H, (int)L, cur_stream()));
  return dq;
}

std::vector<torch::Tensor> masked_pool_fwd(torch::Tensor x,
                                           c10::optional<torch::Tensor> mask) {
  check_bf16(x, "x");
  TORCH_CHECK(x.dim() == 3, "x must be [B, L, D]");
  long B = x.size(0), L = x.size(1), D = x.size(2);
  check_mult8(D, "D");
  const void* mptr = pool_mask_ptr(mask, x, B, L);
  auto pooled = torch::empty({B, D}, x.options());
  auto counts = torch::empty({B}, x.options().dtype(torch::kFloat32));
  auto ws = torch::empty({B, masked_pool_ws_splits(), D},
                         x.options().dtype(torch::kFloat32));
  CHECK_HIP(masked_pool_fwd_launch(x.data_ptr(), mptr, pooled.data_ptr(),
                                   counts.data_ptr(), ws.data_ptr(), (int)B,
                                   (int)L, (int)D, cur_stream()));
  return {pooled, counts};
}

torch::Tensor masked_pool_bwd(torch::Tensor dpooled,
                              c10::optional<torch::Tensor> mask,
                              torch::Tensor counts, long L) {
  check_bf16(dpooled, "dpooled");
  TORCH_CHECK(dpooled.dim() == 2, "dpooled must be [B, D]");
  long B = dpooled.size(0), D = dpooled.size(1);
  check_mult8(D, "D");
  TORCH_CHECK(L > 0, "L must be positive");
  check_f32(counts, "counts");
  check_shape(counts, "counts", {B}, "[B]");
  const void* mptr = pool_mask_ptr(mask, dpooled, B, L);
  auto dx = torch::empty({B, L, D}, dpooled.options());
  CHECK_HIP(masked_pool_bwd_launch(dpooled.data_ptr(), mptr,
                                   counts.data_ptr(), dx.data_ptr(), (int)B,
                                   (int)L, (int)D, cur_stream()));
  return dx;
}

torch::Tensor segment_pool_fwd(torch::Tensor x, torch::Tensor seg_start,
                               torch::Tensor seg_len) {
  check_bf16(x, "x");
  TORCH_CHECK(x.dim() == 2, "x must be [T, D]");
  const long T = x.size(0), D = x.size(1);
  TORCH_CHECK(D % 8 == 0, "D must be a multiple of 8");
  check_i32(seg_start, x, "seg_start");
  check_i32(seg_len, x, "seg_len");
  TORCH_CHECK(seg_start.dim() == 1 && seg_len.dim() == 1 &&
              seg_start.size(0) == seg_len.size(0),
              "seg_start and seg_len must both be [N]");
  const long N = seg_start.size(0);
  auto pooled = torch::empty({N, D}, x.options());
  CHECK_HIP(segment_pool_fwd_launch(x.data_ptr(), seg_start.data_ptr(),
                                    seg_len.data_ptr(), pooled.data_ptr(),
                                    (int)N, T, (int)D, cur_stream()));
  return pooled;
}

torch::Tensor segment_pool_bwd(torch::Tensor dpooled, torch::Tensor pos2seg,
                               torch::Tensor seg_len, long T) {
  check_bf16(dpooled, "dpooled");
  TORCH_CHECK(dpooled.dim() == 2, "dpooled must be [N, D]");
  const long N = dpooled.size(0), D = dpooled.size(1);
  TORCH_CHECK(D % 8 == 0, "D must be a multiple of 8");
  check_i32(pos2seg, dpooled, "pos2seg");
  check_i32(seg_len, dpooled, "seg_len");
  TORCH_CHECK(pos2seg.dim() == 1 && pos2seg.size(0) == T,
              "pos2seg must be [T]");
  TORCH_CHECK(seg_len.dim() == 1 && seg_len.size(0) == N,
              "seg_len must be [N]");
  auto dx = torch::empty({T, D}, dpooled.options());
  CHECK_HIP(segment_pool_bwd_launch(dpooled.data_ptr(), pos2seg.data_ptr(),
                                    seg_len.data_ptr(), dx.data_ptr(), (int)N,
                                    T, (int)D, cur_stream()));
  return dx;
}

torch::Tensor tr_probe(torch::Tensor src, long scheme) {
  check_bf16(src, "src");
  TORCH_CHECK(src.numel() == 256);
  auto out = torch::zeros({64, 4}, src.options());
  CHECK_HIP(tr_probe_launch(src.data_ptr(), out.data_ptr(), (int)scheme,
                            cur_stream()));
  return out;
}

PYBIND11_MODULE(TORCH_EXTENSION_NAME, m) {
  m.def("tr_probe", &tr_probe, "ds_read_b64_tr_b16 semantics probe");
  m.def("masked_pool_fwd", &masked_pool_fwd, "masked mean-pool fwd");
  m.def("masked_pool_bwd", &masked_pool_bwd, "masked mean-pool bwd");
  m.def("segment_pool_fwd", &segment_pool_fwd,
        "per-segment mean-pool fwd (sequence packing)");
  m.def("segment_pool_bwd", &segment_pool_bwd,
        "per-segment mean-pool bwd (sequence packing)");
  m.def("flash_fwd", &flash_fwd,
        "flash attention fwd (gfx950 MFMA, dh=64); seg: optional int32 "
        "[B, L] non-decreasing segment ids, exclusive with mask",
        py::arg("q"), py::arg("k"), py::arg("v"), py::arg("mask"),
        py::arg("scale"), py::arg("seg") = py::none());
  m.def("flash_bwd_fused", &flash_bwd_fused,
        "fused flash bwd: register-accumulated dK/dV (+ optional dS)",
        py::arg("q"), py::arg("k"), py::arg("v"), py::arg("dout"),
        py::arg("mask"), py::arg("lse"), py::arg("ddot"), py::arg("scale"),
        py::arg("emit_ds") = false, py::arg("seg") = py::none());
  m.def("flash_dq_recompute", &flash_dq_recompute,
        "dQ by recompute: S/dP/dS in-register, no dS materialization",
        py::arg("q"), py::arg("k"), py::arg("v"), py::arg("dout"),
        py::arg("mask"), py::arg("lse"), py::arg("ddot"), py::arg("scale"),
        py::arg("seg") = py::none());
  m.def("wgrad_gemm", &wgrad_gemm,
        "split-K wgrad GEMM: dW = dy^T @ x (custom MFMA)",
        py::arg("dy"), py::arg("x"), py::arg("splits") = 0);
  m.def("flash_fwd_packed", &flash_fwd_packed,
        "flash fwd on the packed [B,L,3D] QKV projection output",
        py::arg("qkv"), py::arg("H"), py::arg("mask"), py::arg("scale"),
        py::arg("seg") = py::none());
  m.def("flash_bwd_packed", &flash_bwd_packed,
        "full packed flash bwd: ddot + dK/dV + dQ into one [B,L,3D] grad",
        py::arg("qkv"), py::arg("o"), py::arg("dout"), py::arg("mask"),
        py::arg("lse"), py::arg("H"), py::arg("scale"),
        py::arg("seg") = py::none());
  m.def("flash_bwd_packed_bias", &flash_bwd_packed_bias,
        "flash_bwd_packed plus the column sum of dqkv (qkv bias grad, bf16)",
        py::arg("qkv"), py::arg("o"), py::arg("dout"), py::arg("mask"),
        py::arg("lse"), py::arg("H"), py::arg("scale"),
        py::arg("seg") = py::none());
  m.def("fa_dot", &fa_dot, "rowsum(dO*O) per attention row");
  m.def("flash_dq", &flash_dq, "dQ = dS @ K (MFMA, tr_b16 K^T fragments)");
  m.def("bias_grad", &bias_grad, "bf16 column-sum for linear bias grads");
  m.def("p_from_lse", &p_from_lse, "probabilities from saved logsumexp");
  m.def("qkv_repack", &qkv_repack, "qkv layout repack (fwd/bwd)");
  m.def("qkv_repack_bwd3", &qkv_repack_bwd3, "qkv repack bwd from dq,dk,dv");
  m.def("out_repack", &out_repack, "attention output merge");
  m.def("out_repack_bwd", &out_repack_bwd, "attention output merge bwd");
  m.def("layernorm_fwd", &layernorm_fwd, "fused LayerNorm fwd (bf16, gfx950)");
  m.def("layernorm_bwd", &layernorm_bwd, "fused LayerNorm bwd",
        py::arg("dy"), py::arg("x"), py::arg("gamma"), py::arg("mean"),
        py::arg("rstd"), py::arg("ds_extra"), py::arg("want_dres") = false,
        py::arg("out_bf16") = false);
  m.def("layernorm_drop_fwd", &layernorm_drop_fwd,
        "fused residual dropout + add + LayerNorm fwd",
        py::arg("x"), py::arg("residual"), py::arg("gamma"), py::arg("beta"),
        py::arg("eps"), py::arg("seed"), py::arg("call"), py::arg("site"),
        py::arg("thr"));
  m.def("layernorm_drop_bwd", &layernorm_drop_bwd,
        "fused residual dropout + add + LayerNorm bwd",
        py::arg("dy"), py::arg("x"), py::arg("gamma"), py::arg("mean"),
        py::arg("rstd"), py::arg("ds_extra"), py::arg("out_bf16"),
        py::arg("seed"), py::arg("call"), py::arg("site"), py::arg("thr"));
  m.def("bias_gelu_fwd", &bias_gelu_fwd, "fused bias+GeLU fwd");
  m.def("lt_linear_gelu_bias", &lt_linear_gelu_bias,
        "hipBLASLt GEMM with fused GELU_BIAS epilogue (inference)");
  m.def("lt_bench_algos", &lt_bench_algos,
        "time the heuristic's top algos for a bf16 GEMM config");
  m.def("lt_probe_epilogue", &lt_probe_epilogue,
        "does this hipBLASLt have kernels for (m, n, k, epilogue)?");
  m.def("bias_gelu_bwd", &bias_gelu_bwd, "fused bias+GeLU bwd",
        py::arg("dy"), py::arg("x"), py::arg("b"),
        py::arg("out_bf16") = false);
  m.def("softmax_fwd", &softmax_fwd, "fused scaled masked softmax fwd");
  m.def("softmax_bwd", &softmax_bwd, "fused softmax bwd");
  m.def("adamw_step", &adamw_step, "fused AdamW over flat params");
  m.def("grad_clip_state", &grad_clip_state,
        "deterministic global grad norm -> device {norm, scale, finite, "
        "sumsq}");
  m.def("adamw_step_clipped", &adamw_step_clipped,
        "fused AdamW reading its grad scale / skip flag from clip_state");
}
```

### tosem2021_amd/ops/__init__.py

```python
from __future__ import annotations

from typing import Optional

import torch

from . import reference

_EXT = None
_EXT_ERR: Optional[str] = None


def hip_ops():
    global _EXT, _EXT_ERR
    if _EXT is None:
        try:
            from tosem2021_amd import _hip_ops

            _EXT = _hip_ops
        except ImportError as e:
            _EXT_ERR = str(e)
            raise RuntimeError(
                "tosem2021_amd._hip_ops is not built. On a GPU box this is a "
                "hard error (no eager fallback). Build it in-tree with: "
                "PYTORCH_ROCM_ARCH=gfx950 python setup.py build_ext --inplace "
                f"(import error: {e})"
            ) from e
    return _EXT


def hip_available() -> bool:
    try:
        hip_ops()
        return True
    except RuntimeError:
        return False


class _LayerNormFn(torch.autograd.Function):
    @staticmethod
    def forward(ctx, x, gamma, beta, eps):
        if x.is_cuda:
            y, _, mean, rstd = hip_ops().layernorm_fwd(x, None, gamma, beta, eps)
        else:
            y, mean, rstd = reference.layernorm_fwd(x, gamma, beta, eps)
        ctx.save_for_backward(x, gamma, mean, rstd)
        return y

    @staticmethod
    def backward(ctx, dy):
        x, gamma, mean, rstd = ctx.saved_tensors
        dy = dy.contiguous()
        if x.is_cuda:
            dx, dgamma, dbeta = hip_ops().layernorm_bwd(
                dy, x, gamma, mean, rstd, None, False, True)
            return dx, dgamma, dbeta, None
        dx, dgamma, dbeta = reference.layernorm_bwd(dy, x, gamma, mean, rstd)
        return dx, dgamma.to(gamma.dtype), dbeta.to(gamma.dtype), None


def fused_layernorm(x, gamma, beta, eps: float = 1e-5):
    return _LayerNormFn.apply(x.contiguous(), gamma, beta, eps)


class _AddLayerNormFn(torch.autograd.Function):

    @staticmethod
    def forward(ctx, x, residual, gamma, beta, eps, residual_bias=None):
        ctx.rb_dtype = None if residual_bias is None else residual_bias.dtype
        if x.is_cuda:
            y, s, mean, rstd = hip_ops().layernorm_fwd(x, residual, gamma,
                                                       beta, eps)
        else:
            y, s, mean, rstd = reference.add_layernorm_fwd(x, residual, gamma,
                                                           beta, eps)
        ctx.save_for_backward(s, gamma, mean, rstd)
        return y, s

    @staticmethod
    def backward(ctx, dy, ds):
        s, gamma, mean, rstd = ctx.saved_tensors
        dy = dy.contiguous()
        want_dres = ctx.rb_dtype is not None and ctx.needs_input_grad[5]
        dres = None
        if s.is_cuda:
            de = ds.contiguous() if ds is not None else None
            out = hip_ops().layernorm_bwd(dy, s, gamma, mean, rstd, de,
                                          want_dres, True)
            dx, dgamma, dbeta = out[:3]
            if want_dres:
                dres = out[3].to(ctx.rb_dtype)
            return dx, dx, dgamma, dbeta, None, dres
        dx, dgamma, dbeta = reference.layernorm_bwd(dy, s, gamma, mean, rstd)
        if ds is not None:
            dx = dx + ds
        if want_dres:
            dres = reference.folded_bias_grad(dx).to(ctx.rb_dtype)
        return (dx, dx, dgamma.to(gamma.dtype), dbeta.to(gamma.dtype), None,
                dres)


def fused_add_layernorm(x, residual, gamma, beta, eps: float = 1e-5,
                        residual_bias=None):
    return _AddLayerNormFn.apply(x.contiguous(), residual.contiguous(),
                                 gamma, beta, eps, residual_bias)


class _DropoutAddLayerNormFn(torch.autograd.Function):

    @staticmethod
    def forward(ctx, x, residual, gamma, beta, eps, p, seed, call, site):
        thr, scale = reference.dropout_threshold(p)
        seed, call, site = (seed & 0xFFFFFFFFFFFFFFFF, call & 0xFFFFFFFF,
                            site & 0xFFFFFFFF)
        ctx.drop = (p, seed, call, site, thr, scale)
        if x.is_cuda:
            y, s, mean, rstd = hip_ops().layernorm_drop_fwd(
                x, residual, gamma, beta, eps, seed, call, site, thr)
        else:
            keep = reference.dropout_keep(x.numel() // x.shape[-1],
                                          x.shape[-1], p, seed, call, site)
            y, s, mean, rstd = reference.add_layernorm_fwd(
                x, residual * keep.view(x.shape) * scale, gamma, beta, eps)
        ctx.save_for_backward(s, gamma, mean, rstd)
        return y, s

    @staticmethod
    def backward(ctx, dy, ds):
        s, gamma, mean, rstd = ctx.saved_tensors
        p, seed, call, site, thr, scale = ctx.drop
        dy = dy.contiguous()
        if s.is_cuda:
            de = ds.contiguous() if ds is not None else None
            dx, dres, dgamma, dbeta = hip_ops().layernorm_drop_bwd(
                dy, s, gamma, mean, rstd, de, True, seed, call, site, thr)
            return dx, dres, dgamma, dbeta, None, None, None, None, None
        dx, dgamma, dbeta = reference.layernorm_bwd(dy, s, gamma, mean, rstd)
        if ds is not None:
            dx = dx + ds
        keep = reference.dropout_keep(s.numel() // s.shape[-1], s.shape[-1],
                                      p, seed, call, site)
        dres = dx * keep.view(s.shape) * scale
        return (dx, dres, dgamma.to(gamma.dtype), dbeta.to(gamma.dtype),
                None, None, None, None, None)


def fused_dropout_add_layernorm(x, residual, gamma, beta, eps: float,
                                p: float, seed: int, call: int, site: int):
    reference.dropout_threshold(p)
    return _DropoutAddLayerNormFn.apply(x.contiguous(), residual.contiguous(),
                                        gamma, beta, eps, p, seed, call, site)


class _BiasGeluFn(torch.autograd.Function):
    @staticmethod
    def forward(ctx, x, b):
        ctx.save_for_backward(x, b)
        if x.is_cuda:
            return hip_ops().bias_gelu_fwd(x, b)
        return reference.bias_gelu_fwd(x, b)

    @staticmethod
    def backward(ctx, dy):
        x, b = ctx.saved_tensors
        dy = dy.contiguous()
        if x.is_cuda:
            return tuple(hip_ops().bias_gelu_bwd(dy, x, b, True))
        dx, dbias = reference.bias_gelu_bwd(dy, x, b)
        return dx, dbias.to(b.dtype)


def fused_bias_gelu(x, b):
    return _BiasGeluFn.apply(x.contiguous(), b)


class _SoftmaxFn(torch.autograd.Function):
    @staticmethod
    def forward(ctx, scores, mask, scale):
        if scores.is_cuda:
            p = hip_ops().softmax_fwd(scores, mask, scale)
        else:
            p = reference.softmax_fwd(scores, mask, scale)
        ctx.save_for_backward(p)
        ctx.scale = scale
        return p

    @staticmethod
    def backward(ctx, dp):
        (p,) = ctx.saved_tensors
        dp = dp.contiguous()
        if p.is_cuda:
            ds = hip_ops().softmax_bwd(dp, p, ctx.scale)
        else:
            ds = reference.softmax_bwd(dp, p, ctx.scale)
        return ds, None, None


def fused_softmax(scores, mask=None, scale: float = 1.0):
    return _SoftmaxFn.apply(scores.contiguous(), mask, scale)


class _QkvRepackFn(torch.autograd.Function):

    @staticmethod
    def forward(ctx, qkv, n_heads):
        ctx.n_heads = n_heads
        if qkv.is_cuda:
            stacked = hip_ops().qkv_repack(qkv, n_heads, False)
        else:
            B, L, _ = qkv.shape
            dh = qkv.shape[-1] // (3 * n_heads)
            stacked = (qkv.view(B, L, 3, n_heads, dh).permute(2, 0, 3, 1, 4)
                       .contiguous())
        q, k, v = stacked.unbind(0)
        return q, k, v

    @staticmethod
    def backward(ctx, dq, dk, dv):
        dq = dq.contiguous(); dk = dk.contiguous(); dv = dv.contiguous()
        if dq.is_cuda:
            return hip_ops().qkv_repack_bwd3(dq, dk, dv), None
        B, H, L, dh = dq.shape
        g = torch.stack([dq, dk, dv], dim=0)
        return g.permute(1, 3, 0, 2, 4).reshape(B, L, 3 * H * dh), None


def qkv_repack(qkv, n_heads: int):
    return _QkvRepackFn.apply(qkv.contiguous(), n_heads)


class _OutRepackFn(torch.autograd.Function):

    @staticmethod
    def forward(ctx, x):
        ctx.n_heads = x.shape[1]
        if x.is_cuda:
            return hip_ops().out_repack(x, False)
        B, H, L, dh = x.shape
        return x.permute(0, 2, 1, 3).reshape(B, L, H * dh)

    @staticmethod
    def backward(ctx, g):
        g = g.contiguous()
        if g.is_cuda:
            return hip_ops().out_repack_bwd(g, ctx.n_heads)
        B, L, D = g.shape
        H = ctx.n_heads
        return g.view(B, L, H, D // H).permute(0, 2, 1, 3).contiguous()


def out_repack(x):
    return _OutRepackFn.apply(x.contiguous())


class _LinearFn(torch.autograd.Function):

    @staticmethod
    def forward(ctx, x, w, b):
        ctx.save_for_backward(x, w)
        return torch.addmm(b, x, w.t())

    @staticmethod
    def backward(ctx, dy):
        x, w = ctx.saved_tensors
        dy = dy.contiguous()
        dx = torch.matmul(dy, w)
        dw = torch.matmul(dy.transpose(0, 1), x)
        db = hip_ops().bias_grad(dy) if dy.is_cuda else dy.sum(0)
        return dx, dw, db


def fused_linear(x, w, b):
    lead = x.shape[:-1]
    y = _LinearFn.apply(x.reshape(-1, x.shape[-1]).contiguous(), w, b)
    return y.view(*lead, -1)


class _LinearWgradFn(torch.autograd.Function):

    @staticmethod
    def forward(ctx, x, w, b):
        ctx.save_for_backward(x, w)
        ctx.has_bias = b is not None
        if b is None:
            return torch.matmul(x, w.t())
        return torch.addmm(b, x, w.t())

    @staticmethod
    def backward(ctx, dy):
        x, w = ctx.saved_tensors
        dy = dy.contiguous()
        dx = torch.matmul(dy, w)
        dw = hip_ops().wgrad_gemm(dy, x, 0)
        db = hip_ops().bias_grad(dy) if ctx.has_bias else None
        return dx, dw, db


def wgrad_linear_supported(out_features: int, in_features: int,
                           tokens: int) -> bool:
    return out_features % 256 == 0 and in_features % 256 == 0 and \
        tokens % 32 == 0


def wgrad_linear(x, w, b=None):
    lead = x.shape[:-1]
    y = _LinearWgradFn.apply(x.reshape(-1, x.shape[-1]).contiguous(), w, b)
    return y.view(*lead, -1)


def lt_linear_gelu_bias(x, w1, b1):
    return hip_ops().lt_linear_gelu_bias(x, w1, b1)


class _FlashAttentionFn(torch.autograd.Function):

    @staticmethod
    def forward(ctx, q, k, v, mask, scale, seg=None):
        if q.is_cuda:
            o, lse = hip_ops().flash_fwd(q, k, v, mask, scale, seg)
        else:
            bias = reference.segment_bias(seg) if seg is not None else None
            o, lse = reference.flash_attention_fwd(q, k, v, mask, scale, bias)
        ctx.save_for_backward(q, k, v, o, lse)
        ctx.mask = mask
        ctx.seg = seg
        ctx.scale = scale
        return o

    @staticmethod
    def backward(ctx, do):
        q, k, v, o, lse = ctx.saved_tensors
        mask, seg, scale = ctx.mask, ctx.seg, ctx.scale
        do = do.contiguous()
        if q.is_cuda:
            ddot = hip_ops().fa_dot(do, o)
            dk, dv = hip_ops().flash_bwd_fused(q, k, v, do, mask, lse,
                                               ddot, scale, False, seg)
            dq = hip_ops().flash_dq_recompute(q, k, v, do, mask, lse,
                                              ddot, scale, seg)
            return dq, dk, dv, None, None, None
        bias = reference.segment_bias(seg) if seg is not None else None
        s = torch.matmul(q, k.transpose(-1, -2))
        p = reference.p_from_lse(s, mask, lse, scale, bias)
        dp = torch.matmul(do, v.transpose(-1, -2))
        dsc = reference.softmax_bwd(dp, p, scale)
        dq = torch.matmul(dsc, k)
        dk = torch.matmul(dsc.transpose(-1, -2), q)
        dv = torch.matmul(p.transpose(-1, -2), do)
        return dq, dk, dv, None, None, None


def _check_mask_seg(mask, seg):
    if mask is not None and seg is not None:
        raise ValueError("mask and seg are mutually exclusive: a packed "
                         "batch marks its padding as a trailing segment")


def check_segments(seg: torch.Tensor) -> None:
    if seg.dim() != 2 or seg.dtype not in (torch.int32, torch.int64):
        raise ValueError("seg must be an integer [B, L] tensor")
    if seg.shape[1] > 1:
        bad = (seg[:, 1:] < seg[:, :-1]).any(dim=1)
        if bool(bad.any()):
            rows = torch.nonzero(bad).flatten().tolist()
            raise ValueError(f"seg rows {rows} are not non-decreasing")


def flash_attention(q, k, v, mask=None, scale: float = 1.0, seg=None):
    _check_mask_seg(mask, seg)
    return _FlashAttentionFn.apply(q.contiguous(), k.contiguous(),
                                   v.contiguous(), mask, scale, seg)


class _FlashAttentionPackedFn(torch.autograd.Function):

    @staticmethod
    def forward(ctx, qkv, n_heads, mask, scale, seg=None, qkv_bias=None):
        ctx.qb_dtype = None if qkv_bias is None else qkv_bias.dtype
        if qkv.is_cuda:
            o, lse = hip_ops().flash_fwd_packed(qkv, n_heads, mask, scale,
                                                seg)
        else:
            B, L, D3 = qkv.shape
            d = D3 // 3
            q, k, v = (t.view(B, L, n_heads, 64).transpose(1, 2).contiguous()
                       for t in qkv.split(d, dim=-1))
            bias = reference.segment_bias(seg) if seg is not None else None
            o4, lse = reference.flash_attention_fwd(q, k, v, mask, scale,
                                                    bias)
            o = o4.transpose(1, 2).reshape(B, L, d)
        ctx.save_for_backward(qkv, o, lse)
        ctx.n_heads = n_heads
        ctx.mask = mask
        ctx.seg = seg
        ctx.scale = scale
        return o

    @staticmethod
    def backward(ctx, do):
        qkv, o, lse = ctx.saved_tensors
        n_heads, mask, scale = ctx.n_heads, ctx.mask, ctx.scale
        seg = ctx.seg
        do = do.contiguous()
        want_bias = ctx.qb_dtype is not None and ctx.needs_input_grad[5]
        if qkv.is_cuda:
            if want_bias:
                dqkv, dbias = hip_ops().flash_bwd_packed_bias(
                    qkv, o, do, mask, lse, n_heads, scale, seg)
                return dqkv, None, None, None, None, dbias.to(ctx.qb_dtype)
            dqkv = hip_ops().flash_bwd_packed(qkv, o, do, mask, lse,
                                              n_heads, scale, seg)
            return dqkv, None, None, None, None, None
        bias = reference.segment_bias(seg) if seg is not None else None
        B, L, D3 = qkv.shape
        d = D3 // 3
        q, k, v = (t.view(B, L, n_heads, 64).transpose(1, 2).contiguous()
                   for t in qkv.split(d, dim=-1))
        do4 = do.view(B, L, n_heads, 64).transpose(1, 2).contiguous()
        s = torch.matmul(q, k.transpose(-1, -2))
        p = reference.p_from_lse(s, mask, lse, scale, bias)
        dp = torch.matmul(do4, v.transpose(-1, -2))
        dsc = reference.softmax_bwd(dp, p, scale)
        dq = torch.matmul(dsc, k)
        dk = torch.matmul(dsc.transpose(-1, -2), q)
        dv = torch.matmul(p.transpose(-1, -2), do4)
        dqkv = torch.cat(
            [t.transpose(1, 2).reshape(B, L, d) for t in (dq, dk, dv)],
            dim=-1)
        dbias = None
        if want_bias:
            dbias = reference.folded_bias_grad(dqkv).to(ctx.qb_dtype)
        return dqkv, None, None, None, None, dbias


def flash_attention_packed(qkv, n_heads: int, mask=None, scale: float = 1.0,
                           seg=None, qkv_bias=None):
    _check_mask_seg(mask, seg)
    return _FlashAttentionPackedFn.apply(qkv.contiguous(), n_heads, mask,
                                         scale, seg, qkv_bias)


def flash_supported(head_dim: int, L: int) -> bool:
    return head_dim == 64 and L % 32 == 0


class _MaskedPoolFn(torch.autograd.Function):
    @staticmethod
    def forward(ctx, x, mask):
        if x.is_cuda:
            pooled, counts = hip_ops().masked_pool_fwd(x, mask)
        else:
            if mask is not None:
                w = mask.to(x.dtype).unsqueeze(-1)
                counts = mask.sum(-1).clamp(min=1).float()
                pooled = ((x.float() * w.float()).sum(1) /
                          counts.unsqueeze(-1)).to(x.dtype)
            else:
                counts = torch.full((x.shape[0],), x.shape[1],
                                    dtype=torch.float32)
                pooled = x.float().mean(1).to(x.dtype)
        ctx.save_for_backward(counts)
        ctx.mask = mask
        ctx.L = x.shape[1]
        return pooled

    @staticmethod
    def backward(ctx, dpooled):
        (counts,) = ctx.saved_tensors
        mask = ctx.mask
        dpooled = dpooled.contiguous()
        if dpooled.is_cuda:
            dx = hip_ops().masked_pool_bwd(dpooled, mask, counts, ctx.L)
        else:
            g = (dpooled.float() / counts.unsqueeze(-1)).unsqueeze(1)
            dx = g.expand(-1, ctx.L, -1)
            if mask is not None:
                dx = dx * mask.unsqueeze(-1).float()
            dx = dx.to(dpooled.dtype)
        return dx, None


def masked_mean_pool(x, mask=None):
    return _MaskedPoolFn.apply(x.contiguous(),
                               mask.contiguous() if mask is not None else None)


class _SegmentPoolFn(torch.autograd.Function):
    @staticmethod
    def forward(ctx, x, seg_start, seg_len, pos2seg):
        if x.is_cuda:
            pooled = hip_ops().segment_pool_fwd(x, seg_start, seg_len)
        else:
            pooled = reference.segment_pool_fwd(x, seg_start, seg_len,
                                                pos2seg)
        ctx.save_for_backward(seg_len, pos2seg)
        return pooled

    @staticmethod
    def backward(ctx, dpooled):
        seg_len, pos2seg = ctx.saved_tensors
        dpooled = dpooled.contiguous()
        if dpooled.is_cuda:
            dx = hip_ops().segment_pool_bwd(dpooled, pos2seg, seg_len,
                                            pos2seg.shape[0])
        else:
            dx = reference.segment_pool_bwd(dpooled, seg_len, pos2seg)
        return dx, None, None, None


def segment_mean_pool(x, seg_start, seg_len, pos2seg):
    return _SegmentPoolFn.apply(x.contiguous(), seg_start, seg_len, pos2seg)


def adamw_step(p, grad, m, v, master, *, lr, beta1=0.9, beta2=0.999, eps=1e-8,
               wd=0.01, step, grad_scale=1.0):
    if p.is_cuda:
        hip_ops().adamw_step(p, grad, m, v, master, lr, beta1, beta2, eps, wd,
                             step, grad_scale)
    else:
        reference.adamw_step(p, grad, m, v, master, lr, beta1, beta2, eps, wd,
                             step, grad_scale)


def grad_clip_state(grad, *, grad_scale=1.0, max_norm):
    if not max_norm > 0:
        raise ValueError(f"max_norm must be greater than 0, got {max_norm}")
    if grad.is_cuda:
        return hip_ops().grad_clip_state(grad, grad_scale, max_norm)
    return reference.grad_clip_state(grad, grad_scale, max_norm)


def adamw_step_clipped(p, grad, m, v, master, *, lr, beta1=0.9, beta2=0.999,
                       eps=1e-8, wd=0.01, step, clip_state):
    if p.is_cuda:
        hip_ops().adamw_step_clipped(p, grad, m, v, master, lr, beta1, beta2,
                                     eps, wd, step, clip_state)
    else:
        reference.adamw_step_clipped(p, grad, m, v, master, lr, beta1, beta2,
                                     eps, wd, step, clip_state)
```

### tosem2021_amd/ops/reference.py

```python
from __future__ import annotations

import math
from typing import Optional, Tuple

import numpy as np
import torch


def layernorm_fwd(
    x: torch.Tensor, gamma: torch.Tensor, beta: torch.Tensor, eps: float
) -> Tuple[torch.Tensor, torch.Tensor, torch.Tensor]:
    xf = x.float()
    mean = xf.mean(dim=-1)
    var = xf.var(dim=-1, unbiased=False)
    rstd = torch.rsqrt(var + eps)
    xhat = (xf - mean.unsqueeze(-1)) * rstd.unsqueeze(-1)
    y = xhat * gamma.float() + beta.float()
    return y.to(x.dtype), mean.reshape(-1), rstd.reshape(-1)


def add_layernorm_fwd(x, residual, gamma, beta, eps):
    s = (x.float() + residual.float()).to(x.dtype)
    y, mean, rstd = layernorm_fwd(s, gamma, beta, eps)
    return y, s, mean, rstd


def layernorm_bwd(
    dy: torch.Tensor,
    x: torch.Tensor,
    gamma: torch.Tensor,
    mean: torch.Tensor,
    rstd: torch.Tensor,
) -> Tuple[torch.Tensor, torch.Tensor, torch.Tensor]:
    D = x.shape[-1]
    xf = x.float().reshape(-1, D)
    dyf = dy.float().reshape(-1, D)
    mean = mean.reshape(-1, 1)
    rstd = rstd.reshape(-1, 1)
    xhat = (xf - mean) * rstd
    dyg = dyf * gamma.float()
    c1 = dyg.mean(dim=-1, keepdim=True)
    c2 = (dyg * xhat).mean(dim=-1, keepdim=True)
    dx = rstd * (dyg - c1 - xhat * c2)
    dgamma = (dyf * xhat).sum(dim=0)
    dbeta = dyf.sum(dim=0)
    return dx.reshape(x.shape).to(x.dtype), dgamma, dbeta


def folded_bias_grad(g: torch.Tensor) -> torch.Tensor:
    return g.float().reshape(-1, g.shape[-1]).sum(dim=0)


_PHILOX_M0, _PHILOX_M1 = 0xD2511F53, 0xCD9E8D57
_PHILOX_W0, _PHILOX_W1 = 0x9E3779B9, 0xBB67AE85
_M32 = 0xFFFFFFFF


def philox4x32_10(counter, key) -> np.ndarray:
    c0, c1, c2, c3 = np.broadcast_arrays(
        *(np.asarray(w, dtype=np.uint64) for w in counter))
    k0, k1 = (int(k) & _M32 for k in key)
    m32 = np.uint64(_M32)
    for _ in range(10):
        p0 = np.uint64(_PHILOX_M0) * c0
        p1 = np.uint64(_PHILOX_M1) * c2
        c0, c1, c2, c3 = ((p1 >> np.uint64(32)) ^ c1 ^ np.uint64(k0),
                          p1 & m32,
                          (p0 >> np.uint64(32)) ^ c3 ^ np.uint64(k1),
                          p0 & m32)
        k0 = (k0 + _PHILOX_W0) & _M32
        k1 = (k1 + _PHILOX_W1) & _M32
    return np.stack([c0, c1, c2, c3], axis=-1).astype(np.uint32)


def dropout_threshold(p: float) -> Tuple[int, float]:
    if not 0.0 < p < 1.0:
        raise ValueError(f"dropout probability must be in (0, 1), got {p}")
    thr = min(max(int(math.floor(p * 65536 + 0.5)), 1), 65535)
    return thr, 65536 / (65536 - thr)


def dropout_keep(N: int, D: int, p: float, seed: int, call: int,
                 site: int) -> torch.Tensor:
    if D % 8:
        raise ValueError(f"D must be a multiple of 8, got {D}")
    thr, _ = dropout_threshold(p)
    pkt = np.arange(N * D // 8, dtype=np.uint64)
    words = philox4x32_10(
        (pkt & np.uint64(_M32), pkt >> np.uint64(32), site & _M32,
         call & _M32),
        (seed & _M32, (seed >> 32) & _M32))
    bits = np.stack([words & np.uint32(0xFFFF), words >> np.uint32(16)],
                    axis=-1)
    return torch.from_numpy((bits >= thr).reshape(N, D))


def bias_gelu_fwd(x: torch.Tensor, b: torch.Tensor) -> torch.Tensor:
    pre = x.float() + b.float()
    return torch.nn.functional.gelu(pre, approximate="tanh").to(x.dtype)


def bias_gelu_bwd(
    dy: torch.Tensor, x: torch.Tensor, b: torch.Tensor
) -> Tuple[torch.Tensor, torch.Tensor]:
    pre = (x.float() + b.float()).requires_grad_(True)
    with torch.enable_grad():
        y = torch.nn.functional.gelu(pre, approximate="tanh")
    (dpre,) = torch.autograd.grad(y, pre, dy.float())
    dbias = dpre.reshape(-1, x.shape[-1]).sum(dim=0)
    return dpre.to(x.dtype), dbias


def softmax_fwd(
    scores: torch.Tensor, mask: Optional[torch.Tensor], scale: float
) -> torch.Tensor:
    s = scores.float() * scale
    if mask is not None:
        s = s + mask.float().view(mask.shape[0], 1, 1, mask.shape[-1])
    return torch.softmax(s, dim=-1).to(scores.dtype)


def softmax_bwd(dp: torch.Tensor, p: torch.Tensor, scale: float) -> torch.Tensor:
    dpf = dp.float()
    pf = p.float()
    dot = (dpf * pf).sum(dim=-1, keepdim=True)
    return (scale * pf * (dpf - dot)).to(p.dtype)


def segment_bias(seg: torch.Tensor) -> torch.Tensor:
    same = seg.unsqueeze(-1) == seg.unsqueeze(-2)
    zero = torch.zeros((), dtype=torch.float32, device=seg.device)
    return torch.where(same, zero, zero - 1e9).unsqueeze(1)


def flash_attention_fwd(q, k, v, mask, scale, bias=None):
    s = torch.matmul(q.float(), k.float().transpose(-1, -2)) * scale
    if mask is not None:
        s = s + mask.float().view(mask.shape[0], 1, 1, -1)
    if bias is not None:
        s = s + bias
    lse = torch.logsumexp(s, dim=-1)
    p = torch.softmax(s, dim=-1)
    o = torch.matmul(p, v.float())
    return o.to(q.dtype), lse


def p_from_lse(scores, mask, lse, scale, bias=None):
    s = scores.float() * scale
    if mask is not None:
        s = s + mask.float().view(mask.shape[0], 1, 1, -1)
    if bias is not None:
        s = s + bias
    return torch.exp(s - lse.unsqueeze(-1)).to(scores.dtype)


def segment_pool_fwd(x, seg_start, seg_len, pos2seg):
    n = seg_len.shape[0]
    valid = pos2seg >= 0
    acc = torch.zeros(n, x.shape[-1], dtype=torch.float32, device=x.device)
    acc.index_add_(0, pos2seg[valid].long(), x[valid].float())
    return (acc / seg_len.clamp(min=1).float().unsqueeze(-1)).to(x.dtype)


def segment_pool_bwd(dpooled, seg_len, pos2seg):
    valid = pos2seg >= 0
    idx = pos2seg.clamp(min=0).long()
    g = dpooled.float() / seg_len.clamp(min=1).float().unsqueeze(-1)
    dx = g[idx] * valid.unsqueeze(-1).float()
    return dx.to(dpooled.dtype)


def adamw_step(
    p: torch.Tensor,
    grad: torch.Tensor,
    m: torch.Tensor,
    v: torch.Tensor,
    master: torch.Tensor,
    lr: float,
    beta1: float,
    beta2: float,
    eps: float,
    wd: float,
    step: int,
    grad_scale: float = 1.0,
) -> None:
    g = grad.float() * grad_scale
    m.mul_(beta1).add_(g, alpha=1 - beta1)
    v.mul_(beta2).addcmul_(g, g, value=1 - beta2)
    bc1 = 1.0 / (1.0 - beta1**step)
    bc2 = 1.0 / (1.0 - beta2**step)
    mhat = m * bc1
    vhat = v * bc2
    master.add_(-(lr * (mhat / (vhat.sqrt() + eps) + wd * master)))
    p.copy_(master.to(p.dtype))


def grad_clip_state(grad: torch.Tensor, grad_scale: float,
                    max_norm: float) -> torch.Tensor:
    f32 = torch.float32
    sumsq64 = grad.detach().double().pow(2).sum().cpu()
    sumsq = sumsq64.to(f32)
    gs = torch.tensor(grad_scale, dtype=f32)
    norm = (gs.double() * sumsq64.sqrt()).to(f32)
    ratio = torch.tensor(max_norm, dtype=f32) / (norm + 1e-6)
    one = torch.ones((), dtype=f32)
    coef = torch.where(ratio < 1, ratio, one)
    finite = torch.isfinite(sumsq).to(f32)
    return torch.stack([norm, gs * coef, finite, sumsq]).to(grad.device)


def adamw_step_clipped(p, grad, m, v, master, lr, beta1, beta2, eps, wd,
                       step, clip_state) -> None:
    if float(clip_state[2]) == 0.0:
        return
    adamw_step(p, grad, m, v, master, lr, beta1, beta2, eps, wd, step,
               grad_scale=float(clip_state[1]))
```

Measured before the change: 799,400 tokens/s.

## Skip flash-attention backward query tiles whose output gradient is all zero

The ddot kernel now also emits a per-32-row query-tile flag marking tiles whose dO is entirely ±0. The fused dK/dV kernel uses the flags to jump over dead query tiles, including their prefetch loads. The dQ recompute kernel writes zeros and exits early for fully dead blocks, and skips work per wave otherwise. The skip is exact, since a zero dO gives zero dP, dS and ddot, but it adds a per-tile scan and extra branching, and the ddot kernel is reorganised to one wave per tile.

```diff
diff --git a/csrc/flash_attn.hip b/csrc/flash_attn.hip
--- a/csrc/flash_attn.hip
+++ b/csrc/flash_attn.hip
@@ -221,6 +221,49 @@
   return __builtin_amdgcn_ballot_w64(hit) != 0;
 }
 
+__device__ __forceinline__ unsigned long long fa_live_window(
+    const unsigned char* dead_bh, int t0, int n_t, int lane) {
+  const int t = t0 + lane;
+  bool lv = t < n_t;
+  if (lv && dead_bh) lv = dead_bh[t] == 0;
+  return __builtin_amdgcn_ballot_w64(lv);
+}
+
+__device__ __forceinline__ void fa_store_zero_tile(short* base, int rs, int q0,
+                                                   int L, int lane) {
+#pragma unroll
+  for (int i = 0; i < 4; ++i) {
+    const int row = q0 + 8 * i + (lane >> 3);
+    if (row < L)
+      *(short8_t*)(base + (long)row * rs + (lane & 7) * 8) = (short8_t)(0);
+  }
+}
+
+struct FaLiveScan {
+  const unsigned char* dead_bh;
+  int n_t, lane, win;
+  unsigned long long bits;
+  __device__ __forceinline__ FaLiveScan(const unsigned char* d, int n_t_,
+                                        int lane_)
+      : dead_bh(d), n_t(n_t_), lane(lane_), win(-1), bits(0) {}
+  __device__ __forceinline__ void preload() {
+    if (dead_bh) { win = 0; bits = fa_live_window(dead_bh, 0, n_t, lane); }
+  }
+  __device__ __forceinline__ int next(int qt, int n_q) {
+    if (!dead_bh) return qt;
+    while (qt < n_q) {
+      if ((qt >> 6) != win) {
+        win = qt >> 6;
+        bits = fa_live_window(dead_bh, win << 6, n_t, lane);
+      }
+      const unsigned long long m = bits >> (qt & 63);
+      if (m) return min(qt + (int)__builtin_ctzll(m), n_q);
+      qt = (win + 1) << 6;
+    }
+    return n_q;
+  }
+};
+
 template <bool SEG>
 __global__ void __launch_bounds__(FA_BLOCK, 2)
 flash_fwd_kernel(const short* __restrict__ q, const short* __restrict__ k,
@@ -473,6 +516,7 @@
                        const int* __restrict__ seg,
                        const float* __restrict__ lse,
                        const float* __restrict__ ddot,
+                       const unsigned char* __restrict__ dead,
                        short* __restrict__ ds, short* __restrict__ dk,
                        short* __restrict__ dv,
                        int B, int H, int L, float scale, FaGeom g,
@@ -509,6 +553,10 @@
   int sk = 0;
   if constexpr (SEG) sk = srow[min(my_kv, L - 1)];
 
+  FaLiveScan live(ds == nullptr && dead ? dead + (long)bh * (L / 32) : nullptr,
+                  L / 32, lane);
+  live.preload();
+
   bool skip_tile = false;
   bool wave_skip = false;
   if (mrow && ds == nullptr) {
@@ -550,9 +598,13 @@
     n_q = qr.hi / 32 + 1;
   }
   const FaStager st(tid);
-  short8_t qv8 = st.load(q + qkv_off, qt_begin * 32, g.qkv_rs);
-  short8_t dv8 = st.load(dout + o_off, qt_begin * 32, g.o_rs);
-  for (int qt = qt_begin; qt < n_q; ++qt) {
+  int qt = live.next(qt_begin, n_q), qt_next;
+  short8_t qv8, dv8;
+  if (qt < n_q) {
+    qv8 = st.load(q + qkv_off, qt * 32, g.qkv_rs);
+    dv8 = st.load(dout + o_off, qt * 32, g.o_rs);
+  }
+  for (; qt < n_q; qt = qt_next) {
     const int q0 = qt * 32;
     __syncthreads();
     st.store(q_lds, qv8);
@@ -563,9 +615,10 @@
       if constexpr (SEG) seg_lds[tid] = srow[q0 + tid];
     }
     __syncthreads();
-    if (qt + 1 < n_q) {
-      qv8 = st.load(q + qkv_off, q0 + 32, g.qkv_rs);
-      dv8 = st.load(dout + o_off, q0 + 32, g.o_rs);
+    qt_next = live.next(qt + 1, n_q);
+    if (qt_next < n_q) {
+      qv8 = st.load(q + qkv_off, qt_next * 32, g.qkv_rs);
+      dv8 = st.load(dout + o_off, qt_next * 32, g.o_rs);
     }
 
     if (wave_skip) continue;
@@ -666,7 +719,8 @@
 static void fa_bwd_fused_dispatch(const short* q, const short* k,
                                   const short* v, const void* dout,
                                   const void* mask, const void* seg,
-                                  const void* lse, const void* ddot, void* ds,
+                                  const void* lse, const void* ddot,
+                                  const void* dead, void* ds,
                                   short* dk, short* dv, int B, int H, int L,
                                   float scale, FaGeom g, float* bias_ws,
                                   hipStream_t stream) {
@@ -674,11 +728,12 @@
   const int bias_ld = 3 * H * FA_DH;
 #define FA_BWD_SEG_ARGS                                                       \
   q, k, v, (const short*)dout, nullptr, (const int*)seg, (const float*)lse,   \
-      (const float*)ddot, nullptr, dk, dv, B, H, L, scale, g, bias_ws, bias_ld
+      (const float*)ddot, (const unsigned char*)dead, nullptr, dk, dv, B, H,  \
+      L, scale, g, bias_ws, bias_ld
 #define FA_BWD_ARGS                                                           \
   q, k, v, (const short*)dout, (const float*)mask, nullptr,                   \
-      (const float*)lse, (const float*)ddot, (short*)ds, dk, dv, B, H, L,     \
-      scale, g, bias_ws, bias_ld
+      (const float*)lse, (const float*)ddot, (const unsigned char*)dead,      \
+      (short*)ds, dk, dv, B, H, L, scale, g, bias_ws, bias_ld
   if (seg && bias_ws) {
     flash_bwd_fused_kernel<true, true><<<grid, FA_BLOCK, BWD_SEG_LDS_BYTES,
                                          stream>>>(FA_BWD_SEG_ARGS);
@@ -699,11 +754,11 @@
 extern "C" hipError_t flash_bwd_fused_launch(
     const void* q, const void* k, const void* v, const void* dout,
     const void* mask, const void* seg, const void* lse, const void* ddot,
-    void* ds, void* dk, void* dv, int B, int H, int L, float scale,
-    hipStream_t stream) {
+    const void* dead, void* ds, void* dk, void* dv, int B, int H, int L,
+    float scale, hipStream_t stream) {
   if (seg && ds) return hipErrorInvalidValue;
   fa_bwd_fused_dispatch((const short*)q, (const short*)k, (const short*)v,
-                        dout, mask, seg, lse, ddot, ds, (short*)dk,
+                        dout, mask, seg, lse, ddot, dead, ds, (short*)dk,
                         (short*)dv, B, H, L, scale, FaGeom::bhld(H, L),
                         nullptr, stream);
   return hipGetLastError();
@@ -711,12 +766,12 @@
 
 extern "C" hipError_t flash_bwd_fused_packed_launch(
     const void* qkv, const void* dout, const void* mask, const void* seg,
-    const void* lse, const void* ddot, void* dqkv, void* bias_ws, int B,
-    int H, int L, float scale, hipStream_t stream) {
+    const void* lse, const void* ddot, const void* dead, void* dqkv,
+    void* bias_ws, int B, int H, int L, float scale, hipStream_t stream) {
   const int D = H * FA_DH;
   fa_bwd_fused_dispatch((const short*)qkv, (const short*)qkv + D,
                         (const short*)qkv + 2 * D, dout, mask, seg, lse, ddot,
-                        nullptr, (short*)dqkv + D, (short*)dqkv + 2 * D, B, H,
+                        dead, nullptr, (short*)dqkv + D, (short*)dqkv + 2 * D, B, H,
                         L, scale, FaGeom::packed(H, L), (float*)bias_ws,
                         stream);
   return hipGetLastError();
@@ -812,6 +867,7 @@
                           const int* __restrict__ seg,
                           const float* __restrict__ lse,
                           const float* __restrict__ ddot,
+                          const unsigned char* __restrict__ dead,
                           short* __restrict__ dq,
                           int B, int H, int L, float scale, FaGeom g,
                           float* __restrict__ bias_ws, int bias_ld) {
@@ -832,6 +888,14 @@
   const int h = qb.bh % H;
   const long qkv_off = (long)b * g.qkv_bs + (long)h * g.qkv_hs;
   const long o_off = (long)b * g.o_bs + (long)h * g.o_hs;
+
+  bool tile_dead = false;
+  if (dead) {
+    const int n_t = L / FA_QB;
+    const int t = (qb.qA - wid * FA_QB) / FA_QB + lane;
+    tile_dead = lane < 8 && (t >= n_t || dead[(long)qb.bh * n_t + t] != 0);
+  }
+
   const int my_qA = qb.qA + col;
   const int my_qB = qb.qB + col;
   const bool validA = my_qA < L;
@@ -863,6 +927,23 @@
   const float ddA = ddot[(long)qb.bh * L + (validA ? my_qA : L - 1)];
   const float ddB = ddot[(long)qb.bh * L + (validB ? my_qB : L - 1)];
 
+  const unsigned dmask = (unsigned)__builtin_amdgcn_ballot_w64(tile_dead);
+  if (dmask == 0xffu) {
+    fa_store_zero_tile(dq + qkv_off, g.qkv_rs, qb.qA, L, lane);
+    fa_store_zero_tile(dq + qkv_off, g.qkv_rs, qb.qB, L, lane);
+    if constexpr (BIAS) {
+      if (tid < 2 * FA_DH) {
+        const int n128 = (L + FA_QWG - 1) / FA_QWG;
+        const int blk = (qb.qA - wid * FA_QB) / FA_QWG + tid / FA_DH;
+        if (blk < n128)
+          bias_ws[((long)b * n128 + blk) * bias_ld + h * FA_DH + tid % FA_DH] =
+              0.f;
+      }
+    }
+    return;
+  }
+  const bool wave_dead = ((dmask >> wid) & 0x11u) == 0x11u;
+
   f32x16 dqA[2], dqB[2];
 #pragma unroll
   for (int t = 0; t < 2; ++t) { dqA[t] = (f32x16)(0.f); dqB[t] = (f32x16)(0.f); }
@@ -894,6 +975,7 @@
       kv8 = st.load(k + qkv_off, kv0 + FA_KVB, g.qkv_rs);
       vv8 = st.load(v + qkv_off, kv0 + FA_KVB, g.qkv_rs);
     }
+    if (wave_dead) continue;
 
     float mb_r[16];
     int sk_r[16];
@@ -1000,18 +1082,20 @@
                                      const short* v, const void* dout,
                                      const void* mask, const void* seg,
                                      const void* lse, const void* ddot,
-                                     void* dq, int B, int H, int L,
-                                     float scale, FaGeom g, float* bias_ws,
+                                     const void* dead, void* dq, int B, int H,
+                                     int L, float scale, FaGeom g,
+                                     float* bias_ws,
                                      hipStream_t stream) {
   const dim3 grid = fa_grid(B, H, L, FA_Q2WG);
   const int bias_ld = 3 * H * FA_DH;
 #define FA_DQR_SEG_ARGS                                                       \
   q, k, v, (const short*)dout, nullptr, (const int*)seg, (const float*)lse,   \
-      (const float*)ddot, (short*)dq, B, H, L, scale, g, bias_ws, bias_ld
+      (const float*)ddot, (const unsigned char*)dead, (short*)dq, B, H, L,    \
+      scale, g, bias_ws, bias_ld
 #define FA_DQR_ARGS                                                           \
   q, k, v, (const short*)dout, (const float*)mask, nullptr,                   \
-      (const float*)lse, (const float*)ddot, (short*)dq, B, H, L, scale, g,   \
-      bias_ws, bias_ld
+      (const float*)lse, (const float*)ddot, (const unsigned char*)dead,      \
+      (short*)dq, B, H, L, scale, g, bias_ws, bias_ld
   if (seg && bias_ws) {
     flash_dq_recompute_kernel<true, true><<<grid, FA_BLOCK, DQR_LDS_BYTES,
                                             stream>>>(FA_DQR_SEG_ARGS);
@@ -1032,29 +1116,28 @@
 extern "C" hipError_t flash_dq_recompute_launch(
     const void* q, const void* k, const void* v, const void* dout,
     const void* mask, const void* seg, const void* lse, const void* ddot,
-    void* dq, int B, int H, int L, float scale, hipStream_t stream) {
+    const void* dead, void* dq, int B, int H, int L, float scale,
+    hipStream_t stream) {
   fa_dq_recompute_dispatch((const short*)q, (const short*)k, (const short*)v,
-                           dout, mask, seg, lse, ddot, dq, B, H, L, scale,
+                           dout, mask, seg, lse, ddot, dead, dq, B, H, L, scale,
                            FaGeom::bhld(H, L), nullptr, stream);
   return hipGetLastError();
 }
 
 extern "C" hipError_t flash_dq_recompute_packed_launch(
     const void* qkv, const void* dout, const void* mask, const void* seg,
-    const void* lse, const void* ddot, void* dqkv, void* bias_ws, int B,
-    int H, int L, float scale, hipStream_t stream) {
+    const void* lse, const void* ddot, const void* dead, void* dqkv,
+    void* bias_ws, int B, int H, int L, float scale, hipStream_t stream) {
   const int D = H * FA_DH;
   fa_dq_recompute_dispatch((const short*)qkv, (const short*)qkv + D,
                            (const short*)qkv + 2 * D, dout, mask, seg, lse,
-                           ddot, dqkv, B, H, L, scale, FaGeom::packed(H, L),
+                           ddot, dead, dqkv, B, H, L, scale,
+                           FaGeom::packed(H, L),
                            (float*)bias_ws, stream);
   return hipGetLastError();
 }
 
-__device__ __forceinline__ float fa_row_dot(const short* dr, const short* orow,
-                                            int sub) {
-  short4_t a = *(const short4_t*)(dr + sub * 4);
-  short4_t c = *(const short4_t*)(orow + sub * 4);
+__device__ __forceinline__ float fa_row_dot(short4_t a, short4_t c) {
   float s = 0.f;
 #pragma unroll
   for (int j = 0; j < 4; ++j) s += bf16_to_f32(a[j]) * bf16_to_f32(c[j]);
@@ -1063,50 +1146,82 @@
   return s;
 }
 
-extern "C" __global__ void __launch_bounds__(256)
+__device__ __forceinline__ void fa_dot_tile(const short* dr, const short* orow,
+                                            long rs, float* dd,
+                                            unsigned char* dead_flag,
+                                            int n_valid, int lane) {
+  const int sub = lane & 15, grp = lane >> 4;
+  short4_t a[8], c[8];
+#pragma unroll
+  for (int p = 0; p < 8; ++p) {
+    const int r = min(4 * p + grp, n_valid - 1);
+    a[p] = *(const short4_t*)(dr + r * rs + sub * 4);
+    c[p] = *(const short4_t*)(orow + r * rs + sub * 4);
+  }
+  unsigned nz = 0;
+#pragma unroll
+  for (int p = 0; p < 8; ++p) {
+    const int r = 4 * p + grp;
+    const float s = fa_row_dot(a[p], c[p]);
+    if (r < n_valid) {
+#pragma unroll
+      for (int j = 0; j < 4; ++j) nz |= (unsigned)a[p][j] & 0x7fffu;
+      if (sub == 0) dd[r] = s;
+    }
+  }
+  const bool live = __builtin_amdgcn_ballot_w64(nz != 0) != 0;
+  if (lane == 0) *dead_flag = live ? 0 : 1;
+}
+
+extern "C" __global__ void __launch_bounds__(FA_BLOCK)
 fa_dot_kernel(const short* __restrict__ dout, const short* __restrict__ o,
-              float* __restrict__ ddot, long n_rows) {
-  long row = ((long)blockIdx.x * 256 + threadIdx.x) >> 4;
-  if (row >= n_rows) return;
-  int sub = threadIdx.x & 15;
-  float s = fa_row_dot(dout + row * FA_DH, o + row * FA_DH, sub);
-  if (sub == 0) ddot[row] = s;
-}
-
-extern "C" __global__ void __launch_bounds__(256)
+              float* __restrict__ ddot, unsigned char* __restrict__ dead,
+              long n_rows) {
+  const long tile = (long)blockIdx.x * FA_WAVES + threadIdx.x / WAVE;
+  const long row0 = tile * FA_QB;
+  if (row0 >= n_rows) return;
+  fa_dot_tile(dout + row0 * FA_DH, o + row0 * FA_DH, FA_DH, ddot + row0,
+              dead + tile, (int)min((long)FA_QB, n_rows - row0),
+              threadIdx.x & (WAVE - 1));
+}
+
+extern "C" __global__ void __launch_bounds__(FA_BLOCK)
 fa_dot_packed_kernel(const short* __restrict__ dout,
                      const short* __restrict__ o, float* __restrict__ ddot,
-                     int B, int H, int L) {
+                     unsigned char* __restrict__ dead, int B, int H, int L) {
   const int D = H * FA_DH;
-  long n_rows = (long)B * L * H;
-  long chunk = ((long)blockIdx.x * 256 + threadIdx.x) >> 4;
-  if (chunk >= n_rows) return;
-  int sub = threadIdx.x & 15;
-  int h = (int)(chunk % H);
-  long bl = chunk / H;
-  int l = (int)(bl % L);
-  int b = (int)(bl / L);
-  float s = fa_row_dot(dout + bl * D + h * FA_DH, o + bl * D + h * FA_DH, sub);
-  if (sub == 0) ddot[((long)b * H + h) * L + l] = s;
+  const int n_t = L / FA_QB;
+  const long wv = (long)blockIdx.x * FA_WAVES + threadIdx.x / WAVE;
+  if (wv >= (long)B * n_t * H) return;
+  const int h = (int)(wv % H);
+  const long bt = wv / H;
+  const int t = (int)(bt % n_t);
+  const long b = bt / n_t;
+  const long in_off = (b * L + (long)t * FA_QB) * D + h * FA_DH;
+  const long bh = b * H + h;
+  fa_dot_tile(dout + in_off, o + in_off, D, ddot + bh * L + t * FA_QB,
+              dead + bh * n_t + t, FA_QB, threadIdx.x & (WAVE - 1));
 }
 
 extern "C" hipError_t fa_dot_packed_launch(const void* dout, const void* o,
-                                           void* ddot, int B, int H, int L,
-                                           hipStream_t stream) {
-  long total_threads = (long)B * H * L * 16;
-  int grid = (int)((total_threads + 255) / 256);
-  fa_dot_packed_kernel<<<grid, 256, 0, stream>>>(
-      (const short*)dout, (const short*)o, (float*)ddot, B, H, L);
+                                           void* ddot, void* dead, int B,
+                                           int H, int L, hipStream_t stream) {
+  const long waves = (long)B * H * (L / FA_QB);
+  const int grid = (int)((waves + FA_WAVES - 1) / FA_WAVES);
+  fa_dot_packed_kernel<<<grid, FA_BLOCK, 0, stream>>>(
+      (const short*)dout, (const short*)o, (float*)ddot, (unsigned char*)dead,
+      B, H, L);
   return hipGetLastError();
 }
 
 extern "C" hipError_t fa_dot_launch(const void* dout, const void* o,
-                                    void* ddot, long n_rows,
+                                    void* ddot, void* dead, long n_rows,
                                     hipStream_t stream) {
-  long total_threads = n_rows * 16;
-  int grid = (int)((total_threads + 255) / 256);
-  fa_dot_kernel<<<grid, 256, 0, stream>>>((const short*)dout, (const short*)o,
-                                          (float*)ddot, n_rows);
+  const long waves = (n_rows + FA_QB - 1) / FA_QB;
+  const int grid = (int)((waves + FA_WAVES - 1) / FA_WAVES);
+  fa_dot_kernel<<<grid, FA_BLOCK, 0, stream>>>(
+      (const short*)dout, (const short*)o, (float*)ddot, (unsigned char*)dead,
+      n_rows);
   return hipGetLastError();
 }
 
diff --git a/csrc/launchers.h b/csrc/launchers.h
--- a/csrc/launchers.h
+++ b/csrc/launchers.h
@@ -87,34 +87,35 @@
 hipError_t flash_bwd_fused_launch(const void* q, const void* k, const void* v,
                                   const void* dout, const void* mask,
                                   const void* seg, const void* lse,
-                                  const void* ddot, void* ds, void* dk,
-                                  void* dv, int B, int H, int L, float scale,
-                                  hipStream_t stream);
+                                  const void* ddot, const void* dead,
+                                  void* ds, void* dk, void* dv, int B, int H,
+                                  int L, float scale, hipStream_t stream);
 hipError_t flash_bwd_fused_packed_launch(const void* qkv, const void* dout,
                                          const void* mask, const void* seg,
                                          const void* lse, const void* ddot,
-                                         void* dqkv, void* bias_ws, int B,
-                                         int H, int L, float scale,
-                                         hipStream_t stream);
+                                         const void* dead, void* dqkv,
+                                         void* bias_ws, int B, int H, int L,
+                                         float scale, hipStream_t stream);
 hipError_t flash_dq_recompute_packed_launch(const void* qkv, const void* dout,
                                             const void* mask, const void* seg,
                                             const void* lse, const void* ddot,
-                                            void* dqkv, void* bias_ws, int B,
-                                            int H, int L, float scale,
-                                            hipStream_t stream);
+                                            const void* dead, void* dqkv,
+                                            void* bias_ws, int B, int H, int L,
+                                            float scale, hipStream_t stream);
 int flash_bias_ws_rows(int B, int L);
 hipError_t flash_dq_recompute_launch(const void* q, const void* k,
                                      const void* v, const void* dout,
                                      const void* mask, const void* seg,
                                      const void* lse, const void* ddot,
-                                     void* dq, int B, int H, int L,
-                                     float scale, hipStream_t stream);
+                                     const void* dead, void* dq, int B, int H,
+                                     int L, float scale, hipStream_t stream);
 hipError_t flash_dq_launch(const void* ds, const void* k, void* dq, int B,
                            int H, int L, hipStream_t stream);
 hipError_t fa_dot_launch(const void* dout, const void* o, void* ddot,
-                         long n_rows, hipStream_t stream);
+                         void* dead, long n_rows, hipStream_t stream);
 hipError_t fa_dot_packed_launch(const void* dout, const void* o, void* ddot,
-                                int B, int H, int L, hipStream_t stream);
+                                void* dead, int B, int H, int L,
+                                hipStream_t stream);
 hipError_t tr_probe_launch(const void* src, void* out, int scheme,
                            hipStream_t stream);
 
diff --git a/csrc/ops.cpp b/csrc/ops.cpp
--- a/csrc/ops.cpp
+++ b/csrc/ops.cpp
@@ -525,16 +525,63 @@
   return p;
 }
 
-torch::Tensor fa_dot(torch::Tensor dout, torch::Tensor o) {
+std::vector<torch::Tensor> fa_dot_impl(torch::Tensor dout, torch::Tensor o) {
   check_bf16(dout, "dout"); check_bf16(o, "o");
   TORCH_CHECK(dout.dim() == 4 && o.sizes() == dout.sizes(),
               "dout and o must both be [B, H, L, 64]");
   const long n_rows = dout.numel() / dout.size(-1);
   TORCH_CHECK(dout.size(-1) == 64, "fa_dot expects head_dim 64");
   auto d = torch::empty({n_rows}, dout.options().dtype(torch::kFloat32));
-  CHECK_HIP(fa_dot_launch(dout.data_ptr(), o.data_ptr(), d.data_ptr(), n_rows,
-                          cur_stream()));
-  return d.view({dout.size(0), dout.size(1), dout.size(2)});
+  auto dead = torch::empty({(n_rows + 31) / 32},
+                           dout.options().dtype(torch::kBool));
+  CHECK_HIP(fa_dot_launch(dout.data_ptr(), o.data_ptr(), d.data_ptr(),
+                          dead.data_ptr(), n_rows, cur_stream()));
+  return {d.view({dout.size(0), dout.size(1), dout.size(2)}), dead};
+}
+
+torch::Tensor fa_dot(torch::Tensor dout, torch::Tensor o) {
+  return fa_dot_impl(dout, o)[0];
+}
+
+std::vector<torch::Tensor> fa_dot_flags(torch::Tensor dout, torch::Tensor o) {
+  TORCH_CHECK(dout.dim() == 4 && dout.size(2) % 32 == 0,
+              "fa_dot_flags needs [B, H, L, 64] with L % 32 == 0");
+  auto r = fa_dot_impl(dout, o);
+  return {r[0], r[1].view({dout.size(0), dout.size(1), dout.size(2) / 32})};
+}
+
+std::vector<torch::Tensor> fa_dot_packed_impl(const torch::Tensor& dout,
+                                              const torch::Tensor& o, long B,
+                                              long H, long L) {
+  auto ddot = torch::empty({B, H, L}, dout.options().dtype(torch::kFloat32));
+  auto dead = torch::empty({B, H, L / 32}, dout.options().dtype(torch::kBool));
+  CHECK_HIP(fa_dot_packed_launch(dout.data_ptr(), o.data_ptr(),
+                                 ddot.data_ptr(), dead.data_ptr(), (int)B,
+                                 (int)H, (int)L, cur_stream()));
+  return {ddot, dead};
+}
+
+std::vector<torch::Tensor> fa_dot_packed_flags(torch::Tensor dout,
+                                               torch::Tensor o, long H) {
+  check_bf16(dout, "dout"); check_bf16(o, "o");
+  TORCH_CHECK(dout.dim() == 3 && o.sizes() == dout.sizes() &&
+              dout.size(2) == H * 64 && dout.size(1) % 32 == 0,
+              "dout and o must both be [B, L, H*64] with L % 32 == 0");
+  return fa_dot_packed_impl(dout, o, dout.size(0), H, dout.size(1));
+}
+
+namespace {
+const void* flash_dead_ptr(const c10::optional<torch::Tensor>& dead,
+                           const torch::Tensor& x, const FlashDims& d) {
+  if (!dead.has_value()) return nullptr;
+  TORCH_CHECK(dead->scalar_type() == torch::kBool, "dead must be bool");
+  TORCH_CHECK(dead->device() == x.device() && dead->is_contiguous(),
+              "dead must be contiguous and on the attention inputs' device");
+  TORCH_CHECK(dead->dim() == 3 && dead->size(0) == d.B &&
+              dead->size(1) == d.H && dead->size(2) == d.L / 32,
+              "dead must be [B, H, L / 32]");
+  return dead->data_ptr();
+}
 }
 
 std::vector<torch::Tensor> flash_bwd_fused(torch::Tensor q, torch::Tensor k,
@@ -543,7 +590,8 @@
                                            torch::Tensor lse,
                                            torch::Tensor ddot, double scale,
                                            bool emit_ds,
-                                           c10::optional<torch::Tensor> seg) {
+                                           c10::optional<torch::Tensor> seg,
+                                           c10::optional<torch::Tensor> dead) {
   const auto [B, H, L] = check_flash_bhld(
       "q", q, {{"k", k}, {"v", v}, {"dout", dout}},
       {{"lse", lse}, {"ddot", ddot}});
@@ -551,6 +599,7 @@
   const void* sptr = flash_seg_ptr(seg, mask, q, {B, H, L});
   TORCH_CHECK(!(sptr && emit_ds), "seg with emit_ds=True is not supported: "
               "the flash_dq A/B path is unsegmented");
+  const void* dptr = flash_dead_ptr(dead, q, {B, H, L});
   auto dk = torch::empty_like(k);
   auto dv = torch::empty_like(v);
   torch::Tensor ds;
@@ -561,8 +610,8 @@
   }
   CHECK_HIP(flash_bwd_fused_launch(q.data_ptr(), k.data_ptr(), v.data_ptr(),
                                    dout.data_ptr(), mptr, sptr,
-                                   lse.data_ptr(), ddot.data_ptr(), ds_ptr,
-                                   dk.data_ptr(), dv.data_ptr(), (int)B,
+                                   lse.data_ptr(), ddot.data_ptr(), dptr,
+                                   ds_ptr, dk.data_ptr(), dv.data_ptr(), (int)B,
                                    (int)H, (int)L, (float)scale,
                                    cur_stream()));
   if (emit_ds) return {ds, dk, dv};
@@ -627,16 +676,16 @@
 std::vector<torch::Tensor> flash_bwd_packed_impl(
     torch::Tensor qkv, torch::Tensor o, torch::Tensor dout,
     c10::optional<torch::Tensor> mask, torch::Tensor lse, long H,
-    double scale, c10::optional<torch::Tensor> seg, bool want_bias) {
+    double scale, c10::optional<torch::Tensor> seg, bool want_bias,
+    bool skip_zero_do) {
   const auto dims = check_flash_packed(qkv, H, {{"o", o}, {"dout", dout}},
                                        {{"lse", lse}});
   const long B = dims.B, L = dims.L;
   const void* mptr = flash_mask_ptr(mask, dims);
   const void* sptr = flash_seg_ptr(seg, mask, qkv, dims);
-  auto ddot = torch::empty({B, H, L}, qkv.options().dtype(torch::kFloat32));
-  CHECK_HIP(fa_dot_packed_launch(dout.data_ptr(), o.data_ptr(),
-                                 ddot.data_ptr(), (int)B, (int)H, (int)L,
-                                 cur_stream()));
+  const auto dd = fa_dot_packed_impl(dout, o, B, H, L);
+  const auto& ddot = dd[0];
+  const void* dptr = skip_zero_do ? dd[1].data_ptr() : nullptr;
   auto dqkv = torch::empty_like(qkv);
   torch::Tensor ws;
   void* ws_ptr = nullptr;
@@ -647,11 +696,11 @@
   }
   CHECK_HIP(flash_bwd_fused_packed_launch(
       qkv.data_ptr(), dout.data_ptr(), mptr, sptr, lse.data_ptr(),
-      ddot.data_ptr(), dqkv.data_ptr(), ws_ptr, (int)B, (int)H, (int)L,
+      ddot.data_ptr(), dptr, dqkv.data_ptr(), ws_ptr, (int)B, (int)H, (int)L,
       (float)scale, cur_stream()));
   CHECK_HIP(flash_dq_recompute_packed_launch(
       qkv.data_ptr(), dout.data_ptr(), mptr, sptr, lse.data_ptr(),
-      ddot.data_ptr(), dqkv.data_ptr(), ws_ptr, (int)B, (int)H, (int)L,
+      ddot.data_ptr(), dptr, dqkv.data_ptr(), ws_ptr, (int)B, (int)H, (int)L,
       (float)scale, cur_stream()));
   if (!want_bias) return {dqkv};
   return {dqkv, colsum(ws, ws.size(1), true)};
@@ -663,16 +712,18 @@
                                torch::Tensor dout,
                                c10::optional<torch::Tensor> mask,
                                torch::Tensor lse, long H, double scale,
-                               c10::optional<torch::Tensor> seg) {
-  return flash_bwd_packed_impl(qkv, o, dout, mask, lse, H, scale, seg,
-                               false)[0];
+                               c10::optional<torch::Tensor> seg,
+                               bool skip_zero_do) {
+  return flash_bwd_packed_impl(qkv, o, dout, mask, lse, H, scale, seg, false,
+                               skip_zero_do)[0];
 }
 
 std::vector<torch::Tensor> flash_bwd_packed_bias(
     torch::Tensor qkv, torch::Tensor o, torch::Tensor dout,
     c10::optional<torch::Tensor> mask, torch::Tensor lse, long H,
-    double scale, c10::optional<torch::Tensor> seg) {
-  return flash_bwd_packed_impl(qkv, o, dout, mask, lse, H, scale, seg, true);
+    double scale, c10::optional<torch::Tensor> seg, bool skip_zero_do) {
+  return flash_bwd_packed_impl(qkv, o, dout, mask, lse, H, scale, seg, true,
+                               skip_zero_do);
 }
 
 torch::Tensor flash_dq_recompute(torch::Tensor q, torch::Tensor k,
@@ -680,17 +731,19 @@
                                  c10::optional<torch::Tensor> mask,
                                  torch::Tensor lse, torch::Tensor ddot,
                                  double scale,
-                                 c10::optional<torch::Tensor> seg) {
+                                 c10::optional<torch::Tensor> seg,
+                                 c10::optional<torch::Tensor> dead) {
   const auto [B, H, L] = check_flash_bhld(
       "q", q, {{"k", k}, {"v", v}, {"dout", dout}},
       {{"lse", lse}, {"ddot", ddot}});
   const void* mptr = flash_mask_ptr(mask, {B, H, L});
   const void* sptr = flash_seg_ptr(seg, mask, q, {B, H, L});
+  const void* dptr = flash_dead_ptr(dead, q, {B, H, L});
   auto dq = torch::empty_like(q);
   CHECK_HIP(flash_dq_recompute_launch(q.data_ptr(), k.data_ptr(),
                                       v.data_ptr(), dout.data_ptr(), mptr,
                                       sptr, lse.data_ptr(), ddot.data_ptr(),
-                                      dq.data_ptr(), (int)B, (int)H, (int)L,
+                                      dptr, dq.data_ptr(), (int)B, (int)H, (int)L,
                                       (float)scale, cur_stream()));
   return dq;
 }
@@ -805,12 +858,13 @@
         "fused flash bwd: register-accumulated dK/dV (+ optional dS)",
         py::arg("q"), py::arg("k"), py::arg("v"), py::arg("dout"),
         py::arg("mask"), py::arg("lse"), py::arg("ddot"), py::arg("scale"),
-        py::arg("emit_ds") = false, py::arg("seg") = py::none());
+        py::arg("emit_ds") = false, py::arg("seg") = py::none(),
+        py::arg("dead") = py::none());
   m.def("flash_dq_recompute", &flash_dq_recompute,
         "dQ by recompute: S/dP/dS in-register, no dS materialization",
         py::arg("q"), py::arg("k"), py::arg("v"), py::arg("dout"),
         py::arg("mask"), py::arg("lse"), py::arg("ddot"), py::arg("scale"),
-        py::arg("seg") = py::none());
+        py::arg("seg") = py::none(), py::arg("dead") = py::none());
   m.def("wgrad_gemm", &wgrad_gemm,
         "split-K wgrad GEMM: dW = dy^T @ x (custom MFMA)",
         py::arg("dy"), py::arg("x"), py::arg("splits") = 0);
@@ -822,13 +876,18 @@
         "full packed flash bwd: ddot + dK/dV + dQ into one [B,L,3D] grad",
         py::arg("qkv"), py::arg("o"), py::arg("dout"), py::arg("mask"),
         py::arg("lse"), py::arg("H"), py::arg("scale"),
-        py::arg("seg") = py::none());
+        py::arg("seg") = py::none(), py::arg("skip_zero_do") = true);
   m.def("flash_bwd_packed_bias", &flash_bwd_packed_bias,
         "flash_bwd_packed plus the column sum of dqkv (qkv bias grad, bf16)",
         py::arg("qkv"), py::arg("o"), py::arg("dout"), py::arg("mask"),
         py::arg("lse"), py::arg("H"), py::arg("scale"),
-        py::arg("seg") = py::none());
+        py::arg("seg") = py::none(), py::arg("skip_zero_do") = true);
   m.def("fa_dot", &fa_dot, "rowsum(dO*O) per attention row");
+  m.def("fa_dot_flags", &fa_dot_flags,
+        "fa_dot plus dead [B, H, L/32] bool: query tiles whose dO is all +-0");
+  m.def("fa_dot_packed_flags", &fa_dot_packed_flags,
+        "fa_dot_flags on the packed [B, L, H*64] layout",
+        py::arg("dout"), py::arg("o"), py::arg("H"));
   m.def("flash_dq", &flash_dq, "dQ = dS @ K (MFMA, tr_b16 K^T fragments)");
   m.def("bias_grad", &bias_grad, "bf16 column-sum for linear bias grads");
   m.def("p_from_lse", &p_from_lse, "probabilities from saved logsumexp");
diff --git a/tosem2021_amd/ops/__init__.py b/tosem2021_amd/ops/__init__.py
--- a/tosem2021_amd/ops/__init__.py
+++ b/tosem2021_amd/ops/__init__.py
@@ -1,10 +1,13 @@
 from __future__ import annotations
 
+import os
 from typing import Optional
 
 import torch
 
 from . import reference
+
+_FLASH_QSKIP = os.environ.get("TOSEM_FLASH_QSKIP", "1") != "0"
 
 _EXT = None
 _EXT_ERR: Optional[str] = None
@@ -332,11 +335,13 @@
         mask, seg, scale = ctx.mask, ctx.seg, ctx.scale
         do = do.contiguous()
         if q.is_cuda:
-            ddot = hip_ops().fa_dot(do, o)
+            ddot, dead = hip_ops().fa_dot_flags(do, o)
+            if not _FLASH_QSKIP:
+                dead = None
             dk, dv = hip_ops().flash_bwd_fused(q, k, v, do, mask, lse,
-                                               ddot, scale, False, seg)
+                                               ddot, scale, False, seg, dead)
             dq = hip_ops().flash_dq_recompute(q, k, v, do, mask, lse,
-                                              ddot, scale, seg)
+                                              ddot, scale, seg, dead)
             return dq, dk, dv, None, None, None
         bias = reference.segment_bias(seg) if seg is not None else None
         s = torch.matmul(q, k.transpose(-1, -2))
@@ -405,10 +410,12 @@
         if qkv.is_cuda:
             if want_bias:
                 dqkv, dbias = hip_ops().flash_bwd_packed_bias(
-                    qkv, o, do, mask, lse, n_heads, scale, seg)
+                    qkv, o, do, mask, lse, n_heads, scale, seg,
+                    _FLASH_QSKIP)
                 return dqkv, None, None, None, None, dbias.to(ctx.qb_dtype)
             dqkv = hip_ops().flash_bwd_packed(qkv, o, do, mask, lse,
-                                              n_heads, scale, seg)
+                                              n_heads, scale, seg,
+                                              _FLASH_QSKIP)
             return dqkv, None, None, None, None, None
         bias = reference.segment_bias(seg) if seg is not None else None
         B, L, D3 = qkv.shape
diff --git a/tosem2021_amd/ops/reference.py b/tosem2021_amd/ops/reference.py
--- a/tosem2021_amd/ops/reference.py
+++ b/tosem2021_amd/ops/reference.py
@@ -215,3 +215,24 @@
         return
     adamw_step(p, grad, m, v, master, lr, beta1, beta2, eps, wd, step,
                grad_scale=float(clip_state[1]))
+
+
+def dead_q_tiles(dout: torch.Tensor, n_heads: Optional[int] = None
+                 ) -> torch.Tensor:
+    if dout.dtype != torch.bfloat16:
+        raise ValueError("dead_q_tiles expects bf16")
+    if dout.dim() == 3:
+        B, L, D = dout.shape
+        if n_heads is None or D != n_heads * 64:
+            raise ValueError("packed dout must be [B, L, n_heads * 64]")
+        d4 = dout.view(B, L, n_heads, 64).permute(0, 2, 1, 3)
+    elif dout.dim() == 4 and dout.shape[-1] == 64:
+        d4 = dout
+        B, _, L, _ = dout.shape
+    else:
+        raise ValueError("dout must be [B, L, H * 64] or [B, H, L, 64]")
+    if L % 32:
+        raise ValueError("L % 32 == 0 required")
+    bits = d4.contiguous().view(torch.int16).to(torch.int32) & 0x7FFF
+    live = (bits != 0).view(B, d4.shape[1], L // 32, 32 * 64).any(-1)
+    return ~live
```

New measurement: 809,400 tokens/s, median of 6. 1.2% higher.
